# ppt0011/distributed_training

Measured on AMD Instinct MI355X. Metric: images/sec (node) ResNet-50 at 1/2/4/8 MI355X; grad-sync bus GB/s, higher is better.
Workload: dtype bf16

## Files before the change

distributed_training_amd/_lib.py:

```python
from __future__ import annotations

import ctypes
import os
import threading

import torch

LIB_PATH = os.environ.get(
    "GSYNC_LIB", os.path.join(os.path.dirname(os.path.abspath(__file__)), "lib", "libgsync.so")
)

GS_OK = 0
GS_EINVAL, GS_EHIP, GS_ERCCL, GS_ESTATE, GS_ENOMEM, GS_ENODEV = -1, -2, -3, -4, -5, -6
GS_F32, GS_BF16, GS_F16, GS_F64, GS_I64, GS_I32, GS_U8 = 0, 1, 2, 3, 4, 5, 6
GS_DEV_HOST, GS_DEV_HIP = 0, 1
GS_SUM, GS_PROD, GS_MAX, GS_MIN, GS_AVG = 0, 1, 2, 3, 4
GS_SCALE_NONE, GS_SCALE_MUL, GS_SCALE_DIV = 0, 1, 2
GS_PLAN_SLOTS = 5
GS_RED_GROUPS = 64
GS_RED_PARTIALS = 1024
GS_BKT_AUTO_COLLECTIVE = 1
GS_BKT_GRAD_VIEW = 2
GS_BKT_NO_SCALE = 4
GS_BKT_REDUCE_SCATTER = 8
GS_BKT_NO_UNPACK = 16
GS_LAYOUT_NCHW, GS_LAYOUT_NHWC = 0, 1
GS_OP_PACK, GS_OP_UNPACK, GS_OP_SCALE, GS_OP_SQNORM, GS_OP_UNSCALE, GS_OP_SGD, GS_OP_ADAM, GS_OP_SUM = 1, 2, 3, 4, 5, 6, 7, 8
GS_OP_LARS_NORM, GS_OP_LARS = 9, 10
GS_OP_LAMB_MOMENTS, GS_OP_LAMB = 11, 12
GS_OP_EMA = 13
GS_EMA_EMA, GS_EMA_SWA, GS_EMA_WARMUP = 0, 1, 2

_TORCH_TO_GS = {
    torch.float32: GS_F32,
    torch.bfloat16: GS_BF16,
    torch.float16: GS_F16,
    torch.float64: GS_F64,
    torch.int64: GS_I64,
    torch.int32: GS_I32,
    torch.uint8: GS_U8,
}

_c_int, _c_i64, _c_f, _c_d, _vp = ctypes.c_int, ctypes.c_int64, ctypes.c_float, ctypes.c_double, ctypes.c_void_p
_p_i64 = ctypes.POINTER(ctypes.c_int64)
_p_i32 = ctypes.POINTER(ctypes.c_int32)
_p_u8 = ctypes.POINTER(ctypes.c_uint8)
_p_vp = ctypes.POINTER(ctypes.c_void_p)
_p_f = ctypes.POINTER(ctypes.c_float)

SIGNATURES = {
    "gs_version": (_c_int, []),
    "gs_last_error": (ctypes.c_char_p, []),
    "gs_device_count": (_c_int, []),
    "gs_set_host_threads": (_c_int, [_c_int]),
    "gs_comm_unique_id_bytes": (_c_int, []),
    "gs_comm_get_unique_id": (_c_int, [_p_u8]),
    "gs_comm_create": (_c_int, [_c_int, _c_int, _p_u8, _c_int, _p_vp]),
    "gs_comm_create_ex": (_c_int, [_c_int, _c_int, _p_u8, _c_int, _c_int, _p_vp]),
    "gs_comm_destroy": (_c_int, [_vp]),
    "gs_comm_abort": (_c_int, [_vp]),
    "gs_comm_set_timeout": (_c_int, [_vp, _c_i64]),
    "gs_comm_status": (_c_int, [_vp, ctypes.c_char_p, _c_int]),
    "gs_comm_rank": (_c_int, [_vp]),
    "gs_comm_world": (_c_int, [_vp]),
    "gs_comm_stream": (_c_int, [_vp, _p_vp]),
    "gs_stream_wait": (_c_int, [_vp, _vp]),
    "gs_allreduce": (_c_int, [_vp, _vp, _vp, _c_i64, _c_int, _c_int, _vp]),
    "gs_reduce_scatter": (_c_int, [_vp, _vp, _vp, _c_i64, _c_int, _c_int, _vp]),
    "gs_all_gather": (_c_int, [_vp, _vp, _vp, _c_i64, _c_int, _vp]),
    "gs_broadcast": (_c_int, [_vp, _vp, _vp, _c_i64, _c_int, _c_int, _vp]),
    "gs_allreduce_marked": (_c_int, [_vp, _vp, _vp, _c_i64, _c_int, _c_int, _vp, _vp]),
    "gs_all_gather_marked": (_c_int, [_vp, _vp, _vp, _c_i64, _c_int, _vp, _vp]),
    "gs_plan_create": (_c_int, [_c_int, _c_int, _c_int, _p_i64, _c_i64, _p_vp]),
    "gs_plan_create_ex": (_c_int, [_c_int, _c_int, _c_int, _p_i64, _c_i64, _c_i64, _p_vp]),
    "gs_plan_destroy": (_c_int, [_vp]),
    "gs_plan_flat_numel": (_c_i64, [_vp]),
    "gs_plan_offsets": (_c_int, [_vp, _p_i64]),
    "gs_plan_n_tasks": (_c_int, [_vp]),
    "gs_plan_task_units": (_c_i64, [_vp]),
    "gs_plan_set_hyper_source": (_c_int, [_vp, _vp]),
    "gs_watchdog_pause": (_c_int, [_c_int]),
    "gs_adam_hyper": (_c_int, [_c_int, _vp, _vp, _c_d, _c_d, _c_d, _vp, _vp, _vp]),
    "gs_plan_timer_enable": (_c_int, [_vp, _c_int]),
    "gs_plan_timer_read": (_c_int, [_vp, _p_f, _p_i32, _c_int]),
    "gs_plan_set_ptrs": (_c_int, [_vp, _c_int, _p_vp, _vp]),
    "gs_pack": (_c_int, [_vp, _c_int, _c_int, _vp, _c_int, _c_f, _c_int, _vp]),
    "gs_unpack": (_c_int, [_vp, _vp, _c_int, _c_int, _c_int, _vp, _c_int, _vp]),
    "gs_unpack_check": (_c_int, [_vp, _vp, _c_int, _c_int, _c_int, _vp, _vp]),
    "gs_scale": (_c_int, [_vp, _c_int, _c_int, _c_f, _c_int, _vp]),
    "gs_sqnorm": (_c_int, [_vp, _c_int, _c_int, _vp, _c_int, _vp]),
    "gs_sum": (_c_int, [_vp, _c_int, _c_int, _vp, _c_int, _vp]),
    "gs_sqnorm_partial": (_c_int, [_vp, _c_int, _c_int, _vp]),
    "gs_plan_set_clip": (_c_int, [_vp, _vp, _c_f, _c_f, _c_f, _c_f, _vp]),
    "gs_plan_set_read_hint": (_c_int, [_vp, _c_int]),
    "gs_sqnorm_partial_out": (_c_int, [_vp, _c_int, _c_int, _vp, _p_i32, _vp]),
    "gs_plan_set_clip_groups": (_c_int, [_vp, _vp, ctypes.c_int32, _c_f, _c_f, _c_f, _c_f, _vp]),
    "gs_clip_scale": (_c_int, [_vp, _c_int, _c_int, _vp]),
    "gs_rng_state_bytes": (_c_int, []),
    "gs_rng_draw_u32": (_c_int, [_vp, _c_i64, _c_i64, _vp]),
    "gs_randperm": (_c_int, [ctypes.c_uint64, _c_i64, _vp]),
    "gs_distributed_sampler_indices": (_c_int, [_c_i64, _c_int, _c_int, _c_int, ctypes.c_uint64, _c_i64, _c_int,
                                                _vp, _c_i64, _p_i64]),
    "gs_crop_flip_params": (_c_int, [_vp, _c_i64, _c_int, _c_int, _c_int, _c_int, _c_int, _c_int, _vp, _c_i64,
                                     _vp]),
    "gs_image_augment": (_c_int, [_c_int, _c_int, _vp, _vp, _c_i64, _c_int, _c_int, _c_int, _c_int, _c_int, _c_int,
                                  _vp, _c_i64, _vp, _c_int, _c_int, _vp, _vp]),
    "gs_image_augment_mix": (_c_int, [_c_int, _c_int, _vp, _vp, _c_i64, _c_int, _c_int, _c_int, _c_int, _c_int, _c_int,
                                      _vp, _vp, _c_i64, _vp, _c_int, _c_int, _vp, _vp, _vp, _vp]),
    "gs_bn_bwd_partials": (_c_int, [_c_i64, _c_int]),
    "gs_bn_bwd_reduce": (_c_int, [_vp, _vp, _vp, _vp, _vp, _vp, _c_i64, _c_i64, _c_int, _vp]),
    "gs_bn_bwd_reduce_fork": (_c_int, [_vp, _vp, _vp, _vp, _vp, _vp, _vp, _c_i64, _c_i64, _c_int, _vp]),
    "gs_bn_bwd_dx": (_c_int, [_vp, _vp, _vp, _vp, _vp, _vp, _vp, _c_i64, _vp, _vp, _vp, _c_i64, _c_int, _vp]),
    "gs_add_relu_fwd": (_c_int, [_vp, _vp, _c_i64, _vp]),
    "gs_relu_maxpool_fwd": (_c_int, [_vp, _vp, _vp, _c_i64, _c_int, _c_int, _c_int, _vp]),
    "gs_maxpool_bwd": (_c_int, [_vp, _vp, _vp, _vp, _c_i64, _c_int, _c_int, _c_int, _vp]),
    "gs_relu_mask_fwd": (_c_int, [_vp, _vp, _c_i64, _vp]),
    "gs_add_relu_mask_fwd": (_c_int, [_vp, _vp, _vp, _c_i64, _vp]),
    "gs_relu_maxpool_mask_fwd": (_c_int, [_vp, _vp, _vp, _vp, _c_i64, _c_int, _c_int, _c_int, _vp]),
    "gs_bn_bwd_reduce_bits": (_c_int, [_vp, _vp, _vp, _vp, _vp, _vp, _c_i64, _c_i64, _c_int, _vp]),
    "gs_bn_bwd_reduce_fork_bits": (_c_int, [_vp, _vp, _vp, _vp, _vp, _vp, _vp, _c_i64, _c_i64, _c_int, _vp]),
    "gs_bn_bwd_dx_bits": (_c_int, [_vp, _vp, _vp, _vp, _vp, _vp, _vp, _c_i64, _vp, _vp, _vp, _c_i64, _c_int, _vp]),
    "gs_bn_infer_act": (_c_int, [_vp, _vp, _vp, _vp, _vp, _vp, _c_d, _c_int, _vp, _c_i64, _c_int, _vp]),
    "gs_bn_infer_relu_maxpool": (_c_int, [_vp, _vp, _vp, _vp, _vp, _c_d, _vp, _c_i64, _c_int, _c_int, _c_int, _vp]),
    "gs_eval_accumulate": (_c_int, [_c_int, _vp, _c_int, _vp, _c_i64, _c_i64, _c_i64, _c_i64, _p_i32, _c_int, _c_i64,
                                    _vp, _vp, _vp]),
    "gs_xent_fwd": (_c_int, [_c_int, _vp, _c_int, _vp, _c_i64, _c_i64, _c_i64, _c_i64, _c_f, _vp, _vp, _p_i32, _c_int,
                             _vp, _vp]),
    "gs_xent_bwd": (_c_int, [_c_int, _vp, _c_int, _vp, _c_i64, _c_i64, _c_i64, _c_i64, _c_f, _c_int, _vp, _vp, _vp, _vp,
                             _c_i64, _vp]),
    "gs_xent_mix_fwd": (_c_int, [_c_int, _vp, _c_int, _vp, _vp, _vp, _c_i64, _c_i64, _c_i64, _c_i64, _c_f, _vp, _vp,
                                 _p_i32, _c_int, _vp, _vp]),
    "gs_xent_mix_bwd": (_c_int, [_c_int, _vp, _c_int, _vp, _vp, _vp, _c_i64, _c_i64, _c_i64, _c_i64, _c_f, _c_int, _vp,
                                 _vp, _vp, _vp, _c_i64, _vp]),
    "gs_clip_coef":(_c_int, [_c_int, _vp, _c_f, _c_f, _vp, _vp, _vp]),
    "gs_unscale_check": (_c_int, [_vp, _c_int, _c_int, _vp, _vp, _vp]),
    "gs_sgd_step": (
        _c_int,
        [_vp, _c_int, _c_int, _c_d, _c_d, _c_d, _c_d, _c_int, _c_int, _c_int, _vp, _vp, _vp],
    ),
    "gs_adam_step": (
        _c_int,
        [_vp, _c_int, _c_int, _c_d, _c_d, _c_d, _c_d, _c_d, _c_int, _c_int, _c_d, _c_d, _vp, _vp, _vp],
    ),
    "gs_plan_set_adapt": (_c_int, [_vp, _p_i32]),
    "gs_lars_norms": (_c_int, [_vp, _c_int, _vp, _vp]),
    "gs_lars_step": (_c_int, [_vp, _c_int, _c_d, _c_d, _c_d, _c_d, _c_d, _vp, _vp, _vp, _vp]),
    "gs_lars_step_lowp": (_c_int, [_vp, _c_int, _c_int, _c_d, _c_d, _c_d, _c_d, _c_d, _vp, _vp, _vp, _vp]),
    "gs_lamb_step_lowp": (_c_int, [_vp, _c_int, _c_d, _c_d, _c_d, _c_d, _c_d, _c_d, _c_d, _vp, _vp, _vp]),
    "gs_lamb_moments": (_c_int, [_vp, _c_int, _c_d, _c_d, _c_d, _c_d, _c_d, _c_d, _vp, _vp, _vp, _vp]),
    "gs_lamb_step": (_c_int, [_vp, _c_d, _c_d, _c_d, _c_d, _c_d, _c_d, _c_d, _vp, _vp, _vp]),
    "gs_lamb_hyper": (_c_int, [_c_int, _vp, _vp, _c_d, _c_d, _c_int, _vp, _vp, _vp]),
    "gs_ema_step": (_c_int, [_vp, _c_int, _c_int, _c_d, _c_int, _vp]),
    "gs_ema_hyper": (_c_int, [_c_int, _vp, _c_int, _c_d, _vp, _vp]),
    "gs_compute_bucket_assignment": (
        _c_int,
        [_c_int, _p_i64, _p_i32, _p_i32, _c_int, _p_i64, _p_i32, _p_i32, _p_i32],
    ),
    "gs_bucketer_create": (
        _c_int,
        [_vp, _c_int, _c_int, _c_int, _p_i64, _c_int, _c_int, _p_i32, _p_i32, _c_int, _c_i64, _c_f, _c_int, _p_vp],
    ),
    "gs_bucketer_destroy": (_c_int, [_vp]),
    "gs_bucketer_bucket_numel": (_c_int, [_vp, _c_int, _p_i64]),
    "gs_bucketer_shard_numel": (_c_int, [_vp, _c_int, _p_i64]),
    "gs_bucketer_param_location": (_c_int, [_vp, _c_int, _p_i32, _p_i64]),
    "gs_bucketer_set_bucket_buffer": (_c_int, [_vp, _c_int, _vp]),
    "gs_bucketer_set_shard_buffer": (_c_int, [_vp, _c_int, _vp]),
    "gs_bucketer_prepare": (_c_int, [_vp, _vp]),
    "gs_bucketer_mark_ready": (_c_int, [_vp, _c_int, _vp, _vp, _p_i32, _p_i32]),
    "gs_bucketer_mark_unused": (_c_int, [_vp, _vp, _p_i32, _p_i32]),
    "gs_bucketer_finalize": (_c_int, [_vp, _vp]),
    "gs_bucketer_unpack_bucket": (_c_int, [_vp, _c_int, _vp]),
# ... 158 lines not shown
```

distributed_training_amd/csrc/gs_common.h:

```cpp
#pragma once

#include <cmath>
#include <cstdint>
#include <cstring>
#include <string>
#include <vector>

#include "../../include/gsync.h"
#include "gs_math.h"

namespace gs {

bool roctx_enabled();
void roctx_push(const char* name);
void roctx_pop();
struct GsRange {
  bool on;
  explicit GsRange(const char* name) : on(roctx_enabled()) {
    if (on) roctx_push(name);
  }
  ~GsRange() {
    if (on) roctx_pop();
  }
  GsRange(const GsRange&) = delete;
// ... 248 lines not shown
                        void* stream);
int host_eval_accumulate(const void* logits, int dt, const int64_t* labels, int64_t B, int K, int64_t row_stride,
                         int64_t n_valid, const EvalTopk& topk, int64_t ignore_index, void* ws, void* acc);

struct XentRow {
  float loss, m, logS;
  int32_t code;
};
static_assert(sizeof(XentRow) == 16, "XentRow layout");
struct XentRed {
  float loss_sum, loss_mean;
  int32_t counted, bad;
};
static_assert(sizeof(XentRed) == 16, "XentRed layout");
constexpr int kXentNone = 0, kXentMean = 1, kXentSum = 2;
GS_HD inline float xent_loss(float m, float logS, float zy, float T, int K, float eps) {
  const float nll = (m - zy) + logS;
  if (eps == 0.f) return nll;
  const float smooth = (m + logS) - T / static_cast<float>(K);
  return (1.f - eps) * nll + eps * smooth;
}
GS_HD inline XentRed xent_reduce(double total, int64_t counted, int64_t bad) {
  XentRed r;
  const float nanf32 = static_cast<float>(NAN);
  r.loss_sum = bad ? nanf32 : static_cast<float>(total);
  r.loss_mean = (bad || counted == 0) ? nanf32 : static_cast<float>(total / static_cast<double>(counted));
  r.counted = static_cast<int32_t>(counted);
  r.bad = static_cast<int32_t>(bad);
  return r;
}
GS_HD inline float xent_grad(float z, float m, float logS, float q, float c) {
  const float p = expf((z - m) - logS);
  return c * (p - q);
}
GS_HD inline int32_t xent_mix_code(int64_t a, int64_t b, float lam, int K, int64_t ignore_index) {
  if (a == ignore_index || b == ignore_index) return kEvalSkip;
  if (a < 0 || a >= K || b < 0 || b >= K || !(lam >= 0.f && lam <= 1.f)) return kEvalBad;
  return 0;
}
GS_HD inline bool xent_mix_one(int64_t a, int64_t b, float lam) { return lam == 1.f || a == b; }
GS_HD inline int64_t xent_mix_dominant(int64_t a, int64_t b, float lam) { return lam >= 0.5f ? a : b; }
GS_HD inline float xent_mix_loss(float m, float logS, float za, float zb, float lam, float T, int K, float eps) {
  const float lam1 = 1.f - lam;
  return lam * xent_loss(m, logS, za, T, K, eps) + lam1 * xent_loss(m, logS, zb, T, K, eps);
}
GS_HD inline float xent_mix_q(float eps, float w, float q_off) { return (1.f - eps) * w + q_off; }
int hip_xent_fwd(const void* logits, int dt, const int64_t* labels, int64_t B, int K, int64_t row_stride,
                 int64_t ignore_index, float eps, void* rows, void* red, const EvalTopk& topk, void* acc,
                 void* stream);
int hip_xent_bwd(const void* logits, int dt, const int64_t* labels, int64_t B, int K, int64_t row_stride, float eps,
                 int reduction, const void* rows, const void* red, const float* grad_out, void* dlogits,
                 int64_t d_row_stride, void* stream);
int hip_xent_mix_fwd(const void* logits, int dt, const int64_t* labels_a, const int64_t* labels_b, const float* lam,
                     int64_t B, int K, int64_t row_stride, int64_t ignore_index, float eps, void* rows, void* red,
                     const EvalTopk& topk, void* acc, void* stream);
int host_xent_mix_fwd(const void* logits, int dt, const int64_t* labels_a, const int64_t* labels_b, const float* lam,
                      int64_t B, int K, int64_t row_stride, int64_t ignore_index, float eps, void* rows, void* red,
                      const EvalTopk& topk, void* acc);
int hip_xent_mix_bwd(const void* logits, int dt, const int64_t* labels_a, const int64_t* labels_b, const float* lam,
                     int64_t B, int K, int64_t row_stride, float eps, int reduction, const void* rows, const void* red,
                     const float* grad_out, void* dlogits, int64_t d_row_stride, void* stream);
int host_xent_mix_bwd(const void* logits, int dt, const int64_t* labels_a, const int64_t* labels_b, const float* lam,
                      int64_t B, int K, int64_t row_stride, float eps, int reduction, const void* rows,
                      const void* red, const float* grad_out, void* dlogits, int64_t d_row_stride);

int comm_mark_take(gs_comm* c, void** ev);
bool stream_destroyed(void* stream);
int comm_mark_commit(gs_comm* c, void* ev, void* stream, const gs_plan* consumer);
void comm_forget_consumer(const gs_plan* consumer);

int hip_plan_upload_static(gs_plan* p);
int hip_plan_release(gs_plan* p);
int hip_plan_flush(gs_plan* p, void* stream);
bool stream_capturing(void* stream);
int hip_plan_timer_enable(gs_plan* p, int n_slots);
int hip_plan_timer_read(gs_plan* p, float* ms_out, int32_t* kind_out, int cap);
int hip_pack(gs_plan* p, int src_slot, int src_dt, void* flat, int flat_dt, float s, int mode,
             void* stream);
int hip_unpack(gs_plan* p, const void* flat, int flat_dt, int dst_slot, int dst_dt, float* sq,
               int acc, void* stream);
int hip_unpack_check(gs_plan* p, const void* flat, int flat_dt, int dst_slot, int dst_dt, float* found,
                     void* stream);
int hip_scale(gs_plan* p, int slot, int dt, float s, int mode, void* stream);
int hip_sqnorm(gs_plan* p, int slot, int dt, float* sq, int acc, void* stream);
int hip_sum(gs_plan* p, int slot, int dt, float* out, int acc, void* stream);
int hip_clip_coef(const float* sq, float max_norm, float eps, float* coef, float* norm,
                  void* stream);
int hip_unscale_check(gs_plan* p, int slot, int dt, const float* inv, float* found,
                      void* stream);
int hip_clip_scale(gs_plan* p, int slot, int dt, const ClipArgs& clip, void* stream);
int hip_sqnorm_partial(gs_plan* p, int slot, int dt, float* groups_out, int32_t* n_groups, void* stream);
const float* hip_plan_red_groups(const gs_plan* p);
float* hip_plan_red_scalar(const gs_plan* p);
int hip_sgd(gs_plan* p, int gdt, int ldt, const SgdHyper& h, const float* gs, const float* fi,
            const ClipArgs* clip, void* stream);
int hip_adam(gs_plan* p, int gdt, int ldt, const AdamHyper& h, const float* gs, const float* fi,
             const ClipArgs* clip, void* stream);
int hip_lars_set_adapt(gs_plan* p);
int hip_lars_norms(gs_plan* p, int gdt, float* norms, void* stream);
int hip_lars(gs_plan* p, int gdt, int ldt, const LarsHyper& h, const float* norms, const float* gs, const float* fi,
             void* stream);
int hip_lamb_moments(gs_plan* p, int gdt, const LambHyper& h, float* norms, const float* gs, const float* fi,
                     void* stream);
int hip_lamb(gs_plan* p, int ldt, const LambHyper& h, const float* norms, const float* fi, void* stream);
int hip_lamb_hyper(double* step, const double* lr, double beta1, double beta2, int bias_correction,
                   const float* found_inf, float* hyper, void* stream);
int hip_device_count();
int hip_memset_async(void* dst, int value, size_t bytes, void* stream);
int hip_stream_wait(void* waiter, void* signaler);

int host_pack(gs_plan* p, int src_slot, int src_dt, void* flat, int flat_dt, float s, int mode);
int host_unpack(gs_plan* p, const void* flat, int flat_dt, int dst_slot, int dst_dt, float* sq,
                int acc);
int host_unpack_check(gs_plan* p, const void* flat, int flat_dt, int dst_slot, int dst_dt, float* found);
int host_scale(gs_plan* p, int slot, int dt, float s, int mode);
int host_clip_scale(gs_plan* p, int slot, int dt, const ClipArgs& clip);
int host_sqnorm(gs_plan* p, int slot, int dt, float* sq, int acc);
int host_sum(gs_plan* p, int slot, int dt, float* out, int acc);
int host_clip_coef(const float* sq, float max_norm, float eps, float* coef, float* norm);
int host_unscale_check(gs_plan* p, int slot, int dt, const float* inv, float* found);
int host_sgd(gs_plan* p, int gdt, int ldt, const SgdHyper& h, const float* gs, const float* fi,
             const ClipArgs* clip);
int host_adam(gs_plan* p, int gdt, int ldt, const AdamHyper& h, const float* gs, const float* fi,
              const ClipArgs* clip);
int host_lars_norms(gs_plan* p, int gdt, float* norms);
int host_lars(gs_plan* p, int gdt, int ldt, const LarsHyper& h, const float* norms, const float* gs, const float* fi);
int host_lamb_moments(gs_plan* p, int gdt, const LambHyper& h, float* norms, const float* gs, const float* fi);
int host_lamb(gs_plan* p, int ldt, const LambHyper& h, const float* norms, const float* fi);
float host_clip_factor(const ClipArgs& c, const float* gs);
float host_wave_sum(const float* x, int n, int stride);
}
```

distributed_training_amd/csrc/gs_engine.h:

```cpp

#pragma once

#include <hip/hip_ext.h>
#include <hip/hip_runtime.h>

#include <algorithm>
#include <type_traits>
#include <cmath>
#include <cstdio>
#include <cstdlib>

#include "gs_common.h"

namespace gs {

namespace {

#define HIP_RET(expr)                                                                 \
  do {                                                                                \
    hipError_t _e = (expr);                                                           \
    if (_e != hipSuccess)                                                             \
      return fail(GS_EHIP, std::string(#expr " failed: ") + hipGetErrorString(_e));   \
  } while (0)

// ... 620 lines not shown
  static constexpr int kKind = GS_OP_SQNORM;
  struct Frag { float x[N]; };
  __device__ bool fast_ok(const TV& v) const { return v.vec(0); }
  template <bool F>
  __device__ void load(const TV& v, int64_t e0, uint32_t lo, Frag& f) const {
    ld<DT, N, F, NT>(v.ptr[0], e0, lo, v.numel, v.vec(0), f.x);
  }
  template <bool F>
  __device__ void apply(const TV&, int64_t, uint32_t, Frag& f, float& acc) const {
#pragma unroll
    for (int i = 0; i < N; ++i) acc = fmaf(f.x[i], f.x[i], acc);
  }
};

template <int N, int DT>
struct SumOp : SlotOpBase<N> {
  static constexpr int kG = GS_G_RED;
  static constexpr int kRed = 1;
  static constexpr int kRedGrid = 8192;
  static constexpr int kKind = GS_OP_SUM;
  struct Frag { float x[N]; };
  __device__ bool fast_ok(const TV& v) const { return v.vec(0); }
  template <bool F>
  __device__ void load(const TV& v, int64_t e0, uint32_t lo, Frag& f) const {
    ld<DT, N, F>(v.ptr[0], e0, lo, v.numel, v.vec(0), f.x);
  }
  template <bool F>
  __device__ void apply(const TV&, int64_t, uint32_t, Frag& f, float& acc) const {
#pragma unroll
    for (int i = 0; i < N; ++i) acc += f.x[i];
  }
};

template <int N, int DT>
struct UnscaleOp : SlotOpBase<N> {
  static constexpr int kG = GS_G_RED;
  static constexpr int kRed = 2;
  static constexpr int kRedGrid = 8192;
  static constexpr int kKind = GS_OP_UNSCALE;
  const float* inv;
  struct Frag { float x[N]; };
  __device__ bool fast_ok(const TV& v) const { return v.vec(0); }
  template <bool F>
  __device__ void load(const TV& v, int64_t e0, uint32_t lo, Frag& f) const {
    ld<DT, N, F>(v.ptr[0], e0, lo, v.numel, v.vec(0), f.x);
  }
  template <bool F>
  __device__ void apply(const TV& v, int64_t e0, uint32_t lo, Frag& f, float& acc) const {
#pragma unroll
    for (int i = 0; i < N; ++i)
      if ((F || e0 + lo + i < v.numel) && !isfinite(f.x[i])) acc = 1.f;
    if (inv) {
      const float s = *inv;
      if (s != 1.f) {
#pragma unroll
        for (int i = 0; i < N; ++i) f.x[i] = f.x[i] * s;
        st<DT, N, F>(v.ptr[0], e0, lo, v.numel, v.vec(0), f.x);
      }
    }
  }
};

template <int N, int DT, bool NT = false>
struct ClipScaleOp : SlotOpBase<N> {
  static constexpr int kG = GS_G_UNPACK;
  static constexpr int kKind = GS_OP_SCALE;
  ClipArgs clip{};
  float gsv = 1.f;
  struct Frag { float x[N]; };
  __device__ bool active() const { return gsv != 1.f; }
  __device__ bool fast_ok(const TV& v) const { return v.vec(0); }
  template <bool F>
  __device__ void load(const TV& v, int64_t e0, uint32_t lo, Frag& f) const {
    ld<DT, N, F, NT>(v.ptr[0], e0, lo, v.numel, v.vec(0), f.x);
  }
  template <bool F>
  __device__ void apply(const TV& v, int64_t e0, uint32_t lo, Frag& f, float&) const {
#pragma unroll
    for (int i = 0; i < N; ++i) f.x[i] = f.x[i] * gsv;
    st<DT, N, F>(v.ptr[0], e0, lo, v.numel, v.vec(0), f.x);
  }
};

template <int N, int GD, int LD, bool NTG = true>
struct SgdOp : OpBase<N> {
  static constexpr int kG = GS_G_SGD;
  static constexpr int kKind = GS_OP_SGD;
  SgdHyper h;
  const float* gscale;
  const float* found_inf;
  const float* hyper = nullptr;
  ClipArgs clip{};
  bool clip_on = false;
  bool use_gs = false;
  float gsv = 1.f;
  struct Frag { float p[N], g[N], b[N]; };
  __device__ bool active() const { return found_inf == nullptr || *found_inf == 0.f; }
  __device__ bool fast_ok(const TV& v) const {
    return v.vec(0) && v.vec(1) && (h.mom == 0.f || v.vec(2)) && (LD < 0 || v.vec(3));
  }
  template <bool F>
  __device__ void load(const TV& v, int64_t e0, uint32_t lo, Frag& f) const {
    ld<GS_F32, N, F>(v.ptr[0], e0, lo, v.numel, v.vec(0), f.p);
    ld<GD, N, F, NTG>(v.ptr[1], e0, lo, v.numel, v.vec(1), f.g);
    if (h.mom != 0.f && !h.first) ld<GS_F32, N, F>(v.ptr[2], e0, lo, v.numel, v.vec(2), f.b);
  }
  template <bool F>
  __device__ void apply(const TV& v, int64_t e0, uint32_t lo, Frag& f, float&) const {
#pragma unroll
    for (int i = 0; i < N; ++i) sgd_update(h, use_gs, gsv, f.g[i], &f.p[i], &f.b[i]);
    st<GS_F32, N, F>(v.ptr[0], e0, lo, v.numel, v.vec(0), f.p);
    if (h.mom != 0.f) st<GS_F32, N, F>(v.ptr[2], e0, lo, v.numel, v.vec(2), f.b);
    if constexpr (LD >= 0) st<LD, N, F>(v.ptr[3], e0, lo, v.numel, v.vec(3), f.p);
  }
};

template <int N, int GD, int LD = -1, bool NTG = false>
struct LarsOp : OpBase<N> {
  static constexpr int kG = GS_G_SGD;
  static constexpr int kKind = GS_OP_LARS;
  LarsHyper h;
  const float* norms;
  const int32_t* adapt;
  const float* gscale;
  const float* found_inf;
  const float* hyper = nullptr;
  bool use_gs = false;
  float gsv = 1.f;
  struct Frag { float p[N], g[N], b[N], slr, wd; };
  __device__ bool active() const { return found_inf == nullptr || *found_inf == 0.f; }
  __device__ bool fast_ok(const TV& v) const {
    return v.vec(0) && v.vec(1) && (h.mom == 0.f || v.vec(2)) && (LD < 0 || v.vec(3));
  }
  template <bool F>
  __device__ void load(const TV& v, int64_t e0, uint32_t lo, Frag& f) const {
    ld<GS_F32, N, F>(v.ptr[0], e0, lo, v.numel, v.vec(0), f.p);
    ld<GD, N, F, NTG>(v.ptr[1], e0, lo, v.numel, v.vec(1), f.g);
    if (h.mom != 0.f) ld<GS_F32, N, F>(v.ptr[2], e0, lo, v.numel, v.vec(2), f.b);
    const int t = v.pad;
    lars_coef(h, norms[2 * t], norms[2 * t + 1], adapt[t], use_gs, gsv, &f.slr, &f.wd);
  }
  template <bool F>
  __device__ void apply(const TV& v, int64_t e0, uint32_t lo, Frag& f, float&) const {
#pragma unroll
    for (int i = 0; i < N; ++i) lars_update(h, f.slr, f.wd, use_gs, gsv, f.g[i], &f.p[i], &f.b[i]);
    st<GS_F32, N, F>(v.ptr[0], e0, lo, v.numel, v.vec(0), f.p);
    if (h.mom != 0.f) st<GS_F32, N, F>(v.ptr[2], e0, lo, v.numel, v.vec(2), f.b);
    if constexpr (LD >= 0) st<LD, N, F>(v.ptr[3], e0, lo, v.numel, v.vec(3), f.p);
  }
};

#ifndef GS_G_LAMB
#define GS_G_LAMB 4
#endif
template <int N, int LD = -1>
struct LambOp : OpBase<N> {
  static constexpr int kG = GS_G_LAMB;
  static constexpr int kKind = GS_OP_LAMB;
  LambHyper h;
  const float* norms;
  const int32_t* adapt;
  const float* found_inf;
  const float* hyper = nullptr;
  struct Frag { float p[N], m[N], v[N], slr, wd; };
  __device__ bool active() const { return found_inf == nullptr || *found_inf == 0.f; }
  __device__ bool fast_ok(const TV& tv) const {
// ... 299 lines not shown
```

distributed_training_amd/csrc/gs_host.cpp:

```cpp
#include <algorithm>
#include <atomic>
#include <cmath>
#include <thread>

#include "gs_common.h"

namespace gs {
namespace {

template <int DT>
inline float ldT(const void* base, int64_t i) {
  if constexpr (DT == GS_F32) return static_cast<const float*>(base)[i];
  else return to_f32<DT>(static_cast<const uint16_t*>(base)[i]);
}
template <int DT>
inline void stT(void* base, int64_t i, float v) {
  if constexpr (DT == GS_F32) static_cast<float*>(base)[i] = v;
  else static_cast<uint16_t*>(base)[i] = from_f32<DT>(v);
}
inline void* slot(gs_plan* p, int s, int t) { return p->h_ptrs[static_cast<size_t>(s) * p->n + t]; }

int check_float(int dt) {
  if (!is_float_dtype(dt)) return fail(GS_EINVAL, "unsupported floating dtype");
  return GS_OK;
// ... 27 lines not shown

}

int host_pack(gs_plan* p, int src_slot, int src_dt, void* flat, int flat_dt, float s, int mode) {
  GS_DISPATCH_FLOAT(src_dt, SD, GS_DISPATCH_FLOAT(flat_dt, FD, {
    const int fsz = dtype_size(FD);
    for_ranges(p, [&](int t, int64_t i0, int64_t i1) {
      const void* src = slot(p, src_slot, t);
      void* dst = static_cast<char*>(flat) + p->off[t] * fsz;
      if (!src) {
        const float z = mode == GS_SCALE_MUL ? 0.f * s : (mode == GS_SCALE_DIV ? 0.f / s : 0.f);
        for (int64_t i = i0; i < i1; ++i) stT<FD>(dst, i, z);
      } else if (mode == GS_SCALE_MUL) {
        for (int64_t i = i0; i < i1; ++i) stT<FD>(dst, i, ldT<SD>(src, i) * s);
      } else if (mode == GS_SCALE_DIV) {
        for (int64_t i = i0; i < i1; ++i) stT<FD>(dst, i, round_to<FD>(ldT<SD>(src, i)) / s);
      } else {
        for (int64_t i = i0; i < i1; ++i) stT<FD>(dst, i, ldT<SD>(src, i));
      }
    });
  }));
  return GS_OK;
}

int host_unpack(gs_plan* p, const void* flat, int flat_dt, int dst_slot, int dst_dt, float* sq,
                int acc) {
  GS_DISPATCH_FLOAT(flat_dt, FD, GS_DISPATCH_FLOAT(dst_dt, DD, {
    const int fsz = dtype_size(FD);
    if (sq) {
      double total = 0.0;
      for (int t = 0; t < p->n; ++t) {
        const void* src = static_cast<const char*>(flat) + p->off[t] * fsz;
        void* dst = slot(p, dst_slot, t);
        if (dst == nullptr) continue;
        for (int64_t i = 0; i < p->numel[t]; ++i) {
          const float v = ldT<FD>(src, i);
          stT<DD>(dst, i, v);
          const float r = round_to<DD>(v);
          total += static_cast<double>(r) * r;
        }
      }
      sq[0] = acc ? sq[0] + static_cast<float>(total) : static_cast<float>(total);
    } else {
      for_ranges(p, [&](int t, int64_t i0, int64_t i1) {
        const void* src = static_cast<const char*>(flat) + p->off[t] * fsz;
        void* dst = slot(p, dst_slot, t);
        if (dst == nullptr) return;
        for (int64_t i = i0; i < i1; ++i) stT<DD>(dst, i, ldT<FD>(src, i));
      });
    }
  }));
  return GS_OK;
}

int host_unpack_check(gs_plan* p, const void* flat, int flat_dt, int dst_slot, int dst_dt, float* found) {
  std::atomic<int> bad{found[0] != 0.f ? 1 : 0};
  GS_DISPATCH_FLOAT(flat_dt, FD, GS_DISPATCH_FLOAT(dst_dt, DD, {
    const int fsz = dtype_size(FD);
    for_ranges(p, [&](int t, int64_t i0, int64_t i1) {
      const void* src = static_cast<const char*>(flat) + p->off[t] * fsz;
      void* dst = slot(p, dst_slot, t);
      if (dst == nullptr) return;
      int b = 0;
      for (int64_t i = i0; i < i1; ++i) {
        const float v = ldT<FD>(src, i);
        stT<DD>(dst, i, v);
        b |= !std::isfinite(round_to<DD>(v));
      }
      if (b) bad.store(1);
    });
  }));
  found[0] = bad.load() ? 1.f : 0.f;
  return GS_OK;
}

int host_scale(gs_plan* p, int s_, int dt, float s, int mode) {
  GS_DISPATCH_FLOAT(dt, DT, {
    for_ranges(p, [&](int t, int64_t i0, int64_t i1) {
      void* x = slot(p, s_, t);
      if (mode == GS_SCALE_DIV)
        for (int64_t i = i0; i < i1; ++i) stT<DT>(x, i, ldT<DT>(x, i) / s);
      else
        for (int64_t i = i0; i < i1; ++i) stT<DT>(x, i, ldT<DT>(x, i) * s);
    });
  });
  return GS_OK;
}

int host_clip_scale(gs_plan* p, int s_, int dt, const ClipArgs& clip) {
  const float cf = host_clip_factor(clip, nullptr);
  if (cf == 1.f) return GS_OK;
  return host_scale(p, s_, dt, cf, GS_SCALE_MUL);
}

int host_sqnorm(gs_plan* p, int s_, int dt, float* sq, int acc) {
  GS_DISPATCH_FLOAT(dt, DT, {
    double total = 0.0;
    for (int t = 0; t < p->n; ++t) {
      const void* x = slot(p, s_, t);
      for (int64_t i = 0; i < p->numel[t]; ++i) {
        const double v = ldT<DT>(x, i);
        total += v * v;
      }
    }
    sq[0] = acc ? sq[0] + static_cast<float>(total) : static_cast<float>(total);
  });
  return GS_OK;
}

int host_sum(gs_plan* p, int s_, int dt, float* out, int acc) {
  GS_DISPATCH_FLOAT(dt, DT, {
    double total = 0.0;
    for (int t = 0; t < p->n; ++t) {
      const void* x = slot(p, s_, t);
      for (int64_t i = 0; i < p->numel[t]; ++i) total += ldT<DT>(x, i);
    }
    out[0] = acc ? out[0] + static_cast<float>(total) : static_cast<float>(total);
  });
  return GS_OK;
}

int host_clip_coef(const float* sq, float max_norm, float eps, float* coef, float* norm) {
  const float nrm = sqrtf(sq[0]);
  if (norm) norm[0] = nrm;
  coef[0] = clip_coef(nrm, max_norm, eps, 0);
  return GS_OK;
}

int host_unscale_check(gs_plan* p, int s_, int dt, const float* inv, float* found) {
  std::atomic<int> bad{found[0] != 0.f ? 1 : 0};
  const bool scale = inv && inv[0] != 1.f;
  const float sc = scale ? inv[0] : 1.f;
  GS_DISPATCH_FLOAT(dt, DT, {
    for_ranges(p, [&](int t, int64_t i0, int64_t i1) {
      void* x = slot(p, s_, t);
      int b = 0;
      for (int64_t i = i0; i < i1; ++i) {
        const float v = ldT<DT>(x, i);
        b |= !std::isfinite(v);
        if (scale) stT<DT>(x, i, v * sc);
      }
      if (b) bad.store(1);
    });
  });
  found[0] = bad.load() ? 1.f : 0.f;
  return GS_OK;
}

float host_wave_sum(const float* x, int n, int stride) {
  float v[64], t[64];
  for (int l = 0; l < 64; ++l) {
    float a = 0.f;
    for (int j = l; j < n; j += 64) a = a + x[static_cast<int64_t>(j) * stride];
    v[l] = 0.f + a;
  }
  auto step = [&](auto src, unsigned row_mask) {
    for (int l = 0; l < 64; ++l) t[l] = ((row_mask >> (l >> 4)) & 1u) ? v[src(l)] : 0.f;
    for (int l = 0; l < 64; ++l) v[l] = v[l] + t[l];
  };
  static const int q1[4] = {1, 0, 3, 2}, q2[4] = {2, 3, 0, 1};
  step([](int l) { return (l & ~3) | q1[l & 3]; }, 0xFu);
  step([](int l) { return (l & ~3) | q2[l & 3]; }, 0xFu);
  step([](int l) { return (l & ~7) | (7 - (l & 7)); }, 0xFu);
  step([](int l) { return (l & ~15) | (15 - (l & 15)); }, 0xFu);
  step([](int l) { return (l & ~15) - 1; }, 0xAu);
  step([](int) { return 31; }, 0xCu);
// ... 431 lines not shown
```

distributed_training_amd/csrc/gs_kernels.hip:

```cpp

#include "gs_engine.h"

namespace gs {

int hip_device_count() {
  int n = 0;
  if (hipGetDeviceCount(&n) != hipSuccess) return 0;
  return n;
}

int hip_memset_async(void* dst, int value, size_t bytes, void* stream) {
  HIP_RET(hipMemsetAsync(dst, value, bytes, static_cast<hipStream_t>(stream)));
  return GS_OK;
}

int hip_stream_wait(void* waiter, void* signaler) {
  if (waiter == signaler) return GS_OK;
  hipEvent_t ev;
  HIP_RET(hipEventCreateWithFlags(&ev, hipEventDisableTiming));
  hipError_t e1 = hipEventRecord(ev, static_cast<hipStream_t>(signaler));
  hipError_t e2 = e1 == hipSuccess ? hipStreamWaitEvent(static_cast<hipStream_t>(waiter), ev, 0)
                                   : e1;
  (void)hipEventDestroy(ev);
  if (e2 != hipSuccess) return fail(GS_EHIP, std::string("stream wait: ") + hipGetErrorString(e2));
// ... 160 lines not shown
  HIP_RET(hipMemcpyAsync(p->d_table, stage, tb, hipMemcpyHostToDevice, s));
  HIP_RET(hipEventRecord(static_cast<hipEvent_t>(p->ring_events[k]), s));
  p->ring = (k + 1) & 3;
  p->dirty = false;
  return GS_OK;
}

constexpr int64_t kPackG2MaxChunks = 4096;

template <int SD, int FD, int MODE, bool NT>
static int pack_mode(gs_plan* p, int src_slot, void* flat, float s, void* stream) {
  if constexpr (FD == GS_F32) {
    if (static_cast<int64_t>(p->chunks.size()) <= kPackG2MaxChunks) {
      PackOp<kUnit, SD, FD, MODE, NT, true> op;
      op.slot = src_slot; op.flat = flat; op.flat_vec = flat_aligned(flat); op.s = s;
      return launch(p, op, stream);
    }
  }
  PackOp<kUnit, SD, FD, MODE, NT> op;
  op.slot = src_slot; op.flat = flat; op.flat_vec = flat_aligned(flat); op.s = s;
  return launch(p, op, stream);
}

template <bool NT>
static int pack_nt(gs_plan* p, int src_slot, int src_dt, void* flat, int flat_dt, float s, int mode,
                   void* stream) {
  GS_DISPATCH_FLOAT(src_dt, SD, GS_DISPATCH_FLOAT(flat_dt, FD, {
    switch (mode) {
      case GS_SCALE_NONE: return pack_mode<SD, FD, GS_SCALE_NONE, NT>(p, src_slot, flat, s, stream);
      case GS_SCALE_MUL: return pack_mode<SD, FD, GS_SCALE_MUL, NT>(p, src_slot, flat, s, stream);
      case GS_SCALE_DIV: return pack_mode<SD, FD, GS_SCALE_DIV, NT>(p, src_slot, flat, s, stream);
      default: return fail(GS_EINVAL, "gs_pack: unknown scale mode");
    }
  }));
  return GS_OK;
}

int hip_pack(gs_plan* p, int src_slot, int src_dt, void* flat, int flat_dt, float s, int mode,
             void* stream) {
  DeviceGuard g(p->device);
  return nt_read_once(p->elems * dtype_bytes(src_dt))
             ? pack_nt<true>(p, src_slot, src_dt, flat, flat_dt, s, mode, stream)
             : pack_nt<false>(p, src_slot, src_dt, flat, flat_dt, s, mode, stream);
}

template <int RED, bool NT>
static int unpack_nt(gs_plan* p, const void* flat, int flat_dt, int dst_slot, int dst_dt, float* red, int acc,
                     void* stream) {
  GS_DISPATCH_FLOAT(flat_dt, FD, GS_DISPATCH_FLOAT(dst_dt, DD, {
    UnpackOp<kUnit, FD, DD, RED, NT> op;
    op.want_red = red != nullptr; op.flat = flat; op.flat_vec = flat_aligned(flat); op.slot = dst_slot;
    return launch(p, op, stream, red, acc);
  }));
  return GS_OK;
}

int hip_unpack(gs_plan* p, const void* flat, int flat_dt, int dst_slot, int dst_dt, float* sq,
               int acc, void* stream) {
  DeviceGuard g(p->device);
  return nt_read_once(p->flat_numel * dtype_bytes(flat_dt))
             ? unpack_nt<1, true>(p, flat, flat_dt, dst_slot, dst_dt, sq, acc, stream)
             : unpack_nt<1, false>(p, flat, flat_dt, dst_slot, dst_dt, sq, acc, stream);
}

int hip_unpack_check(gs_plan* p, const void* flat, int flat_dt, int dst_slot, int dst_dt, float* found,
                     void* stream) {
  DeviceGuard g(p->device);
  return nt_read_once(p->flat_numel * dtype_bytes(flat_dt))
             ? unpack_nt<2, true>(p, flat, flat_dt, dst_slot, dst_dt, found, 1, stream)
             : unpack_nt<2, false>(p, flat, flat_dt, dst_slot, dst_dt, found, 1, stream);
}

int hip_scale(gs_plan* p, int slot, int dt, float s, int mode, void* stream) {
  DeviceGuard g(p->device);
  GS_DISPATCH_FLOAT(dt, DT, {
    ScaleOp<kUnit, DT> op;
    op.slot = slot; op.s = s; op.mode = mode;
    return launch(p, op, stream);
  });
  return GS_OK;
}

template <bool NT>
static int sqnorm_nt(gs_plan* p, int slot, int dt, float* sq, int acc, int groups_only, void* stream) {
  GS_DISPATCH_FLOAT(dt, DT, {
    SqnormOp<kUnit, DT, NT> op;
    op.slot = slot;
    return launch(p, op, stream, sq, acc, groups_only);
  });
  return GS_OK;
}
static int sqnorm_launch(gs_plan* p, int slot, int dt, float* sq, int acc, int groups_only, void* stream) {
  if (!nt_read_once(p->elems * dtype_bytes(dt), true, p->read_hint))
    return sqnorm_nt<false>(p, slot, dt, sq, acc, groups_only, stream);
  p->grads_read = false;
  return sqnorm_nt<true>(p, slot, dt, sq, acc, groups_only, stream);
}

int hip_sqnorm(gs_plan* p, int slot, int dt, float* sq, int acc, void* stream) {
  DeviceGuard g(p->device);
  return sqnorm_launch(p, slot, dt, sq, acc, 0, stream);
}

const float* hip_plan_red_groups(const gs_plan* p) {
  return p->d_partials + kGridLimit + kRedSyncWords + kRedSyncStride;
}
float* hip_plan_red_scalar(const gs_plan* p) { return p->d_partials + kGridLimit + kRedSyncWords; }

int hip_sqnorm_partial(gs_plan* p, int slot, int dt, float* groups_out, int32_t* n_groups, void* stream) {
  DeviceGuard g(p->device);
  const bool own = groups_out == nullptr;
  if (own) groups_out = const_cast<float*>(hip_plan_red_groups(p));
  if (!own && p->elems > 0 &&
      static_cast<int64_t>(p->chunks.size()) <= kRawChunksMax) {
    GS_TRY_RET(sqnorm_launch(p, slot, dt, groups_out, 0, 2, stream));
    if (n_groups) *n_groups = p->red_groups;
    p->red_valid = false;
    p->red_groups = 0;
    return GS_OK;
  }
  const int cap = std::min(p->grid_cap, red_grid_cap(SqnormOp<kUnit, GS_F32>::kRedGrid));
  const bool groups = p->elems > 0 &&
                      red_fuse_groups() > 0 && cap <= kRedFuseMaxGrid;
  if (groups) {
    GS_TRY_RET(sqnorm_launch(p, slot, dt, groups_out, 0, 1, stream));
    if (n_groups) *n_groups = p->red_groups;
    return GS_OK;
  }
  p->red_groups = 0;
  if (n_groups) *n_groups = 1;
  GS_TRY_RET(sqnorm_launch(p, slot, dt, hip_plan_red_scalar(p), 0, 0, stream));
  if (!own) {
    HIP_RET(hipMemsetAsync(groups_out, 0, GS_RED_PARTIALS * sizeof(float), static_cast<hipStream_t>(stream)));
    HIP_RET(hipMemcpyAsync(groups_out, hip_plan_red_scalar(p), sizeof(float), hipMemcpyDeviceToDevice,
                           static_cast<hipStream_t>(stream)));
  }
  return GS_OK;
}

int hip_sum(gs_plan* p, int slot, int dt, float* out, int acc, void* stream) {
  DeviceGuard g(p->device);
  GS_DISPATCH_FLOAT(dt, DT, {
    SumOp<kUnit, DT> op;
    op.slot = slot;
    return launch(p, op, stream, out, acc);
  });
  return GS_OK;
}

int hip_clip_coef(const float* sq, float max_norm, float eps, float* coef, float* norm,
                  void* stream) {
  hipLaunchKernelGGL(clip_coef_kernel, dim3(1), dim3(64), 0, static_cast<hipStream_t>(stream),
                     sq, max_norm, eps, coef, norm);
  HIP_RET(hipGetLastError());
  return GS_OK;
}

__global__ void adam_hyper_kernel(double* step, const double* lr, double beta1, double beta2, double wd,
                                  const float* found_inf, float* hyper) {
  if (threadIdx.x == 0) adam_hyper_update(step, lr, beta1, beta2, wd, found_inf, hyper);
}

int hip_adam_hyper(double* step, const double* lr, double beta1, double beta2, double wd,
                   const float* found_inf, float* hyper, void* stream) {
  hipLaunchKernelGGL(adam_hyper_kernel, dim3(1), dim3(64), 0, static_cast<hipStream_t>(stream), step, lr,
                     beta1, beta2, wd, found_inf, hyper);
// ... 47 lines not shown
```

distributed_training_amd/csrc/gs_plan.cpp:

```cpp
#include <algorithm>
#include <cstdlib>
#include <map>
#include <new>

#include <rocprofiler-sdk-roctx/roctx.h>

#include "gs_common.h"

namespace gs {

static thread_local std::string g_last_error;

bool roctx_enabled() {
  static const bool on = [] {
    const char* e = std::getenv("GSYNC_ROCTX");
    return e && std::atoi(e) != 0;
  }();
  return on;
}
void roctx_push(const char* name) { roctxRangePushA(name); }
void roctx_pop() { roctxRangePop(); }

void set_error(const std::string& msg) { g_last_error = msg; }
int fail(int code, const std::string& msg) {
// ... 180 lines not shown
  std::copy(p->off.begin(), p->off.end(), out);
  return GS_OK;
}

int gs_plan_n_tasks(gs_plan* p) { return p ? p->n_tasks : -1; }

int64_t gs_plan_task_units(gs_plan* p) { return p ? p->task_units : -1; }

int gs_plan_timer_enable(gs_plan* p, int n_slots) {
  GS_CHECK_ARG(p != nullptr, "gs_plan_timer_enable: NULL plan");
  GS_CHECK_ARG(n_slots >= 0 && n_slots <= 4096, "gs_plan_timer_enable: n_slots out of [0, 4096]");
  if (p->kind != GS_DEV_HIP) return fail(GS_EINVAL, "gs_plan_timer_enable: host plans have no launch timer");
  return hip_plan_timer_enable(p, n_slots);
}

int gs_plan_timer_read(gs_plan* p, float* ms_out, int32_t* kind_out, int cap) {
  GS_CHECK_ARG(p != nullptr && (cap == 0 || ms_out != nullptr), "gs_plan_timer_read: NULL argument");
  if (p->kind != GS_DEV_HIP) return fail(GS_EINVAL, "gs_plan_timer_read: host plans have no launch timer");
  return hip_plan_timer_read(p, ms_out, kind_out, cap);
}

int gs_plan_set_ptrs(gs_plan* p, int slot, void* const* ptrs, void* ) {
  GS_CHECK_ARG(p != nullptr, "gs_plan_set_ptrs: NULL plan");
  GS_CHECK_ARG(slot >= 0 && slot < GS_PLAN_SLOTS, "gs_plan_set_ptrs: slot out of range");
  GS_CHECK_ARG(p->n == 0 || ptrs != nullptr, "gs_plan_set_ptrs: NULL ptrs");
  void** row = p->h_ptrs.data() + static_cast<size_t>(slot) * p->n;
  for (int t = 0; t < p->n; ++t) {
    if (row[t] != ptrs[t]) {
      row[t] = ptrs[t];
      const uint32_t bit = 1u << slot;
      const bool al = (reinterpret_cast<uintptr_t>(ptrs[t]) & 15u) == 0;
      p->h_align[t] = al ? (p->h_align[t] | bit) : (p->h_align[t] & ~bit);
      p->dirty = true;
    }
  }
  return GS_OK;
}

#define PLAN_OK(p) GS_CHECK_ARG((p) != nullptr, "NULL plan")
#define SLOT_OK(s) GS_CHECK_ARG((s) >= 0 && (s) < GS_PLAN_SLOTS, "slot out of range")

int gs_pack(gs_plan* p, int src_slot, int src_dtype, void* flat, int flat_dtype, float scale,
            int scale_mode, void* stream) {
  GsRange range("gs_pack");
  PLAN_OK(p);
  SLOT_OK(src_slot);
  GS_CHECK_ARG(flat != nullptr || p->flat_numel == 0, "gs_pack: NULL flat buffer");
  GS_CHECK_ARG(scale_mode >= GS_SCALE_NONE && scale_mode <= GS_SCALE_DIV, "gs_pack: bad scale_mode");
  if (p->kind == GS_DEV_HOST) return host_pack(p, src_slot, src_dtype, flat, flat_dtype, scale, scale_mode);
  return hip_pack(p, src_slot, src_dtype, flat, flat_dtype, scale, scale_mode, stream);
}

int gs_unpack(gs_plan* p, const void* flat, int flat_dtype, int dst_slot, int dst_dtype,
              float* sqnorm_dev, int accumulate, void* stream) {
  GsRange range("gs_unpack");
  PLAN_OK(p);
  SLOT_OK(dst_slot);
  GS_CHECK_ARG(flat != nullptr || p->flat_numel == 0, "gs_unpack: NULL flat buffer");
  if (p->kind == GS_DEV_HOST)
    return host_unpack(p, flat, flat_dtype, dst_slot, dst_dtype, sqnorm_dev, accumulate);
  return hip_unpack(p, flat, flat_dtype, dst_slot, dst_dtype, sqnorm_dev, accumulate, stream);
}

int gs_unpack_check(gs_plan* p, const void* flat, int flat_dtype, int dst_slot, int dst_dtype,
                    float* found_inf, void* stream) {
  GsRange range("gs_unpack_check");
  PLAN_OK(p);
  SLOT_OK(dst_slot);
  GS_CHECK_ARG(flat != nullptr || p->flat_numel == 0, "gs_unpack_check: NULL flat buffer");
  GS_CHECK_ARG(found_inf != nullptr, "gs_unpack_check: NULL found_inf");
  if (p->kind == GS_DEV_HOST) return host_unpack_check(p, flat, flat_dtype, dst_slot, dst_dtype, found_inf);
  return hip_unpack_check(p, flat, flat_dtype, dst_slot, dst_dtype, found_inf, stream);
}

int gs_scale(gs_plan* p, int slot, int dtype, float s, int scale_mode, void* stream) {
  GsRange range("gs_scale");
  PLAN_OK(p);
  SLOT_OK(slot);
  GS_CHECK_ARG(scale_mode == GS_SCALE_MUL || scale_mode == GS_SCALE_DIV, "gs_scale: bad scale_mode");
  if (p->kind == GS_DEV_HOST) return host_scale(p, slot, dtype, s, scale_mode);
  return hip_scale(p, slot, dtype, s, scale_mode, stream);
}

int gs_sqnorm(gs_plan* p, int slot, int dtype, float* sqnorm_dev, int accumulate, void* stream) {
  GsRange range("gs_sqnorm");
  PLAN_OK(p);
  SLOT_OK(slot);
  GS_CHECK_ARG(sqnorm_dev != nullptr, "gs_sqnorm: NULL output");
  p->grads_read = slot == 1;
  if (p->kind == GS_DEV_HOST) return host_sqnorm(p, slot, dtype, sqnorm_dev, accumulate);
  return hip_sqnorm(p, slot, dtype, sqnorm_dev, accumulate, stream);
}

int gs_sqnorm_partial(gs_plan* p, int slot, int dtype, void* stream) {
  GsRange range("gs_sqnorm_partial");
  PLAN_OK(p);
  SLOT_OK(slot);
  p->red_valid = true;
  p->grads_read = slot == 1;
  if (p->kind == GS_DEV_HOST) {
    p->red_groups = 0;
    return host_sqnorm(p, slot, dtype, &p->h_red, 0);
  }
  return hip_sqnorm_partial(p, slot, dtype, nullptr, nullptr, stream);
}

int gs_sqnorm_partial_out(gs_plan* p, int slot, int dtype, float* groups_out, int32_t* n_groups,
                          void* stream) {
  GsRange range("gs_sqnorm_partial_out");
  PLAN_OK(p);
  SLOT_OK(slot);
  GS_CHECK_ARG(groups_out != nullptr && n_groups != nullptr, "gs_sqnorm_partial_out: NULL argument");
  p->red_valid = true;
  p->grads_read = slot == 1;
  if (p->kind == GS_DEV_HOST) {
    p->red_groups = 0;
    GS_TRY_RET(host_sqnorm(p, slot, dtype, &p->h_red, 0));
    groups_out[0] = p->h_red;
    std::fill(groups_out + 1, groups_out + GS_RED_PARTIALS, 0.f);
    *n_groups = 1;
    return GS_OK;
  }
  return hip_sqnorm_partial(p, slot, dtype, groups_out, n_groups, stream);
}

int gs_plan_set_read_hint(gs_plan* p, int hint) {
  PLAN_OK(p);
  GS_CHECK_ARG(hint >= 0 && hint <= 2, "gs_plan_set_read_hint: hint 0, 1 or 2");
  p->read_hint = hint;
  return GS_OK;
}

int gs_plan_set_clip(gs_plan* p, const float* sqnorm_dev, float max_norm, float eps, float sq_mul,
                     float coef_mul, float* out_dev) {
  PLAN_OK(p);
  if (!(max_norm > 0.f)) {
    p->clip_on = false;
    return GS_OK;
  }
  GS_CHECK_ARG(eps >= 0.f, "gs_plan_set_clip: eps < 0");
  p->clip_on = true;
  p->clip_own = sqnorm_dev == nullptr;
  p->clip = ClipArgs{sqnorm_dev, 0, 1, max_norm, eps, sq_mul, coef_mul, out_dev};
  return GS_OK;
}

int gs_plan_set_clip_groups(gs_plan* p, const float* groups_dev, int32_t n_groups, float max_norm,
                            float eps, float sq_mul, float coef_mul, float* out_dev) {
  PLAN_OK(p);
  if (!(max_norm > 0.f)) {
    p->clip_on = false;
    return GS_OK;
  }
  GS_CHECK_ARG(groups_dev != nullptr, "gs_plan_set_clip_groups: NULL group sums");
  GS_CHECK_ARG(n_groups >= 1 && n_groups <= GS_RED_PARTIALS, "gs_plan_set_clip_groups: n_groups out of 1..GS_RED_PARTIALS");
  GS_CHECK_ARG(eps >= 0.f, "gs_plan_set_clip_groups: eps < 0");
  p->clip_on = true;
  p->clip_own = false;
  p->clip = ClipArgs{groups_dev, n_groups, 1, max_norm, eps, sq_mul, coef_mul, out_dev};
  return GS_OK;
}

static int plan_clip(gs_plan* p, ClipArgs* c, const ClipArgs** out) {
  *out = nullptr;
  if (!p->clip_on) return GS_OK;
  *c = p->clip;
// ... 370 lines not shown
```

distributed_training_amd/csrc/gs_torch_hook.cpp:

```cpp
#include <pybind11/pybind11.h>
#include <pybind11/stl.h>
#include <torch/csrc/autograd/engine.h>
#include <torch/csrc/autograd/function.h>
#include <torch/csrc/autograd/function_hook.h>
#include <torch/csrc/autograd/variable.h>
#include <torch/csrc/utils/pybind.h>

#include <ATen/hip/impl/HIPStreamMasqueradingAsCUDA.h>
#include <c10/hip/HIPStream.h>

#include <algorithm>
#include <memory>
#include <stdexcept>
#include <string>
#include <vector>

#include "../../include/gsync.h"

namespace py = pybind11;
using torch::autograd::Node;
using torch::autograd::variable_list;

namespace {

// ... 119 lines not shown
    }
    const int bk = bucket_of_[i];
    held_[bk].push_back(g);
    p.mutable_grad() = at::Tensor();
    int32_t n_ready = 0;
    const int rc = gs_bucketer_mark_ready(b_, i, g.data_ptr(), stream_, ready_.data(), &n_ready);
    if (rc < 0) throw std::runtime_error(std::string("gs_bucketer_mark_ready: ") + gs_last_error());
    for (int k = 0; k < n_ready; ++k) {
      auto& hs = held_[ready_[k]];
      if (comm_stream_ != nullptr) {
        const c10::Stream cs = c10::hip::getStreamFromExternalMasqueradingAsCUDA(
            static_cast<hipStream_t>(comm_stream_), static_cast<c10::DeviceIndex>(device_));
        for (auto& t : hs) t.record_stream(cs);
      }
      hs.clear();
    }
  }

  void set_mark_unused(bool on) { mark_unused_ = on; }

  void finalize() {
    if (mark_unused_) {
      int32_t n_ready = 0;
      const int ru = gs_bucketer_mark_unused(b_, stream_, ready_.data(), &n_ready);
      if (ru < 0) {
        in_backward_ = false;
        finalize_queued_ = false;
        pinned_.clear();
        throw std::runtime_error(std::string("gs_bucketer_mark_unused: ") + gs_last_error());
      }
    }
    const int rc = gs_bucketer_finalize(b_, stream_);
    in_backward_ = false;
    finalize_queued_ = false;
    pinned_.clear();
    if (rc < 0) throw std::runtime_error(std::string("gs_bucketer_finalize: ") + gs_last_error());
    std::string err;
    const PyGILState_STATE st = PyGILState_Ensure();
    PyObject* r = PyObject_CallObject(on_finalize_, nullptr);
    if (r == nullptr) {
      PyObject *t, *v, *tb;
      PyErr_Fetch(&t, &v, &tb);
      PyObject* sv = v ? PyObject_Str(v) : nullptr;
      const char* msg = sv ? PyUnicode_AsUTF8(sv) : nullptr;
      err = msg ? msg : "error in the DDP finalize callback";
      Py_XDECREF(sv);
      Py_XDECREF(t);
      Py_XDECREF(v);
      Py_XDECREF(tb);
      PyErr_Clear();
    }
    Py_XDECREF(r);
    PyGILState_Release(st);
    if (!err.empty()) throw std::runtime_error(err);
  }

  std::vector<int> order() const { return order_; }
  bool in_backward() const { return in_backward_; }
  bool finalize_queued() const { return finalize_queued_; }
  uintptr_t stream() const { return reinterpret_cast<uintptr_t>(stream_); }

 private:
  std::vector<at::Tensor> params_;
  int device_;
  PyObject* on_finalize_;
  std::vector<std::weak_ptr<Node>> accs_;
  std::vector<std::shared_ptr<Node>> pinned_;
  std::vector<uintptr_t> keys_;
  bool active_ = false;
  std::vector<std::vector<int64_t>> dense_strides_;
  std::vector<char> dense_seen_;
  gs_bucketer* b_ = nullptr;
  std::vector<int32_t> ready_;
  void* stream_ = nullptr;
  bool in_backward_ = false, finalize_queued_ = false, record_order_ = false;
  bool release_ = false;
  bool mark_unused_ = false;
  std::vector<int> bucket_of_;
  std::vector<std::vector<at::Tensor>> held_;
  void* comm_stream_ = nullptr;
  std::vector<int> order_;
};

variable_list MarkReady::operator()(const variable_list& outputs, const variable_list& ) {
  owner->on_grad(index);
  return outputs;
}

}

PYBIND11_MODULE(_gshook, m) {
  m.doc() = "libgsync DDP gradient hooks in C++ (AccumulateGrad post-hooks -> gs_bucketer_mark_ready)";
  py::class_<Hooks, std::shared_ptr<Hooks>>(m, "Hooks")
      .def(py::init<std::vector<at::Tensor>, int, py::function, bool>(), py::arg("params"), py::arg("device"),
           py::arg("on_finalize"), py::arg("release") = false)
      .def("attach", &Hooks::attach)
      .def("detach", &Hooks::detach)
      .def("attached", &Hooks::attached)
      .def("set_bucketer", &Hooks::set_bucketer, py::arg("handle"), py::arg("n_buckets"),
           py::arg("bucket_of") = std::vector<int>(), py::arg("comm_stream") = 0)
      .def("set_mark_unused", &Hooks::set_mark_unused)
      .def("prepare", &Hooks::prepare)
      .def("order", &Hooks::order)
      .def("in_backward", &Hooks::in_backward)
      .def("finalize_queued", &Hooks::finalize_queued)
      .def("stream", &Hooks::stream);
}
```

distributed_training_amd/ddp.py:

```python
from __future__ import annotations

import ctypes
import os
import sys
from contextlib import contextmanager
from dataclasses import dataclass
from enum import Enum, auto
from typing import Any, Callable

import torch
import torch.distributed as dist
import torch.nn as nn
from torch.distributed.algorithms.join import Join, Joinable, JoinHook

from . import _lib as L
from .comm import get_communicator
from .multi_tensor import TensorListPlan, dense_like_param, is_dense

DEFAULT_FIRST_BUCKET_BYTES = getattr(dist, "_DEFAULT_FIRST_BUCKET_BYTES", 1024 * 1024)
BUCKET_ALIGN_ELEMS = 64


def compute_bucket_assignment_by_size(tensors, size_limits, order=None):
    n = len(tensors)
    nbytes = L.i64_array([t.numel() * t.element_size() for t in tensors])
    keys = []
    key_ids: dict = {}
    for t in tensors:
        k = (t.dtype, t.device)
        keys.append(key_ids.setdefault(k, len(key_ids)))
    limits = [int(min(x, 2**62)) for x in size_limits]
    bucket_of = (ctypes.c_int32 * max(1, n))()
    members = (ctypes.c_int32 * max(1, n))()
    counts = (ctypes.c_int32 * max(1, n))()
    nb = L.check(
        L.lib().gs_compute_bucket_assignment(
            n, nbytes, L.i32_array(keys), None if order is None else L.i32_array(order), len(limits),
            L.i64_array(limits), bucket_of, members, counts),
        "gs_compute_bucket_assignment",
    )
    out, pos = [], 0
    for b in range(nb):
        out.append([int(members[pos + k]) for k in range(counts[b])])
        pos += counts[b]
    return out


def split_last_bucket(buckets, nbytes, cap):
    if not buckets:
        return buckets
    last = list(buckets[-1])
    tail, size = [], 0
    while last and (not tail or size + nbytes[last[-1]] <= cap):
        i = last.pop()
        tail.insert(0, i)
        size += nbytes[i]
    out = [list(b) for b in buckets[:-1]]
    if last:
        out.append(last)
    out.append(tail)
    return out


def xgmi_bucket_caps(allreduce_time, world: int, sizes_mib=(1, 4, 16, 64), efficiency: float = 0.85) -> dict:
    f = 2.0 * (world - 1) / world
    pts = [(m * 1024 * 1024, allreduce_time(m * 1024 * 1024)) for m in sizes_mib]
    n = len(pts)
    sx = sum(p[0] for p in pts)
    sy = sum(p[1] for p in pts)
    sxx = sum(p[0] * p[0] for p in pts)
    sxy = sum(p[0] * p[1] for p in pts)
    beta = (n * sxy - sx * sy) / max(1e-30, n * sxx - sx * sx)
    alpha = max(0.0, (sy - beta * sx) / n)
    if beta <= 0:
        beta = pts[-1][1] / pts[-1][0]
    bus = f / beta
    cap = efficiency / (1 - efficiency) * alpha * bus / f
    cap = int(min(256 * 2**20, max(4 * 2**20, cap)))
    last = int(min(cap, max(256 * 1024, alpha * bus / f)))
    return {"points": [{"bytes": b, "ms": t * 1e3, "bus_GBps": b * f / t / 1e9} for b, t in pts],
            "alpha_us": alpha * 1e6, "bus_GBps": bus / 1e9, "bucket_cap_bytes": cap, "last_bucket_cap_bytes": last,
            "efficiency": efficiency}


def _as_words(t: torch.Tensor):
    if not t.is_contiguous():
        return None
    if t.dtype in (torch.float32, torch.bfloat16, torch.float16):
        return t
    if t.element_size() in (4, 8) and t.dtype != torch.complex64:
        return t.reshape(-1).view(torch.float32)
    return None


class GradBucket:

    def __init__(self, index, buffer, params, offsets, is_last):
        self._index = index
# ... 192 lines not shown
        self.device_ids = device_ids if device_ids is None else [torch.device(d).index if not isinstance(d, int) else d for d in device_ids]
        self.output_device = output_device
        dtypes = {p.dtype for p in self._params}
        if not all(dt.is_floating_point for dt in dtypes):
            raise NotImplementedError(f"gradient sync needs floating parameters, got {dtypes}")
        self._bucket_dtype_override = bucket_dtype
        self._grad_dtype = self._params[0].dtype if len(dtypes) == 1 else None
        self._bucket_dtype = bucket_dtype if bucket_dtype is not None else self._grad_dtype
        if self.device.type == "cuda":
            self._dev_index = self.device.index if self.device.index is not None else torch.cuda.current_device()
            if not L.available():
                raise L.GsyncUnavailable(L._load_error)
        else:
            self._dev_index = 0
        self._backend = dist.get_backend(self.process_group)

        self._comm = None
        self._own_comm = False
        if self.device.type == "cuda" and collective != "process_group" and self._backend == "nccl":
            pg = None if self.process_group is dist.group.WORLD else self.process_group
            if rccl_max_ctas:
                from .comm import Communicator

                self._comm = Communicator(pg, torch.device("cuda", self._dev_index), max_ctas=int(rccl_max_ctas))
                self._own_comm = True
            else:
                self._comm = get_communicator(pg, torch.device("cuda", self._dev_index))
        self._comm_hook: tuple[Any, Callable] | None = None
        self._buffers_plan = None
        self._sqnorm_target: torch.Tensor | None = None
        self._sqnorm_valid = False
        self._sqnorm_versions = None
        self._found_inf_target: torch.Tensor | None = None
        self._found_inf_valid = False

        self._debug_sums = None
        if os.environ.get("GSYNC_DEBUG", "0") not in ("", "0"):
            self._debug_sums = torch.zeros(0)

        if init_sync:
            self._verify_param_shape_across_processes()
            self._sync_module_states()

        if bucket_policy not in ("torch", "xgmi"):
            raise ValueError(f"bucket_policy must be 'torch' or 'xgmi', got {bucket_policy!r}")
        self.bucket_policy = bucket_policy
        self._last_bucket_cap = None if last_bucket_cap_mb is None else int(last_bucket_cap_mb * 1024 * 1024)
        self._xgmi_calibration = None
        if bucket_policy == "xgmi" and self.world_size > 1:
            cal = xgmi_bucket_caps(self._calib_allreduce, self.world_size)
            self._xgmi_calibration = cal
            if bucket_cap_mb is None:
                self.bucket_bytes_cap = cal["bucket_cap_bytes"]
            if last_bucket_cap_mb is None:
                self._last_bucket_cap = cal["last_bucket_cap_bytes"]

        if static_graph or not find_unused_parameters:
            limits = [sys.maxsize]
        elif self.bucket_bytes_cap_default:
            limits = [DEFAULT_FIRST_BUCKET_BYTES, self.bucket_bytes_cap]
        else:
            limits = [self.bucket_bytes_cap]
        buckets = compute_bucket_assignment_by_size(self._params, limits)
        self._bucketer = self._make_bucketer(list(reversed(buckets)))
        self._has_rebuilt_buckets = False
        self._ready_order: list[int] = []
        self._in_backward = False
        self._finalize_queued = False
        self._stream = None
        self._pending: dict[int, Any] = {}
        self._num_iterations = 0
        self._capture_local: dict | None = None
        self._used_local = [0] * len(self._params) if find_unused_parameters else None
        self._ready_now: list = []
        self._overlap: dict | None = None
        self._param_index = {id(p): i for i, p in enumerate(self._params)}
        self._hook_handles = []
        self._native = _make_native_hooks(self) if self.device.type == "cuda" else None
        self._native_on = False
        if self._native is not None:
            self._native.set_bucketer(self._bucketer.handle.value, len(self._bucketer.buckets))
            self._native.set_mark_unused(bool(self.static_graph))
        self._set_native(self._native_ok())

    def _flags(self):
        flags = 0
        if self._comm is not None and self._comm_hook is None:
            flags |= L.GS_BKT_AUTO_COLLECTIVE
        if self.gradient_as_bucket_view:
            flags |= L.GS_BKT_GRAD_VIEW
        if self._comm_hook is not None:
            flags |= L.GS_BKT_NO_SCALE
        return flags

    def _make_bucketer(self, buckets):
        old = getattr(self, "_bucketer", None)
        if old is not None:
            old.close()
        b = _Bucketer(self, buckets, self._flags())
        self._div_factor = float(self.world_size)
        t = getattr(self, "_found_inf_target", None)
        if t is not None:
            L.check(L.lib().gs_bucketer_set_found_inf(b.handle, t.data_ptr()), "gs_bucketer_set_found_inf")
        if getattr(self, "_debug_sums", None) is not None:
            self._debug_sums = torch.zeros(3 * len(buckets), dtype=torch.float32, device=self.device)
            L.check(L.lib().gs_bucketer_set_debug(b.handle, self._debug_sums.data_ptr()), "gs_bucketer_set_debug")
        lvl = getattr(self, "_timeline", None)
        if lvl is not None:
            L.check(L.lib().gs_bucketer_set_timeline(b.handle, lvl), "gs_bucketer_set_timeline")
        if getattr(self, "_overlap", None) is not None:
            self._overlap["per_bucket"] = {}
        if getattr(self, "_native", None) is not None:
            self._native.set_bucketer(b.handle.value, len(buckets))
        return b

    def _native_ok(self) -> bool:
        return (self._native is not None and bool(self._bucketer.flags & L.GS_BKT_AUTO_COLLECTIVE)
                and not self.find_unused_parameters and self._overlap is None and self._comm_hook is None
                and self._capture_local is None)

    def _set_native(self, on: bool):
        if on:
            for h in self._hook_handles:
                h.remove()
            self._hook_handles = []
            self._native.attach()
        else:
            if self._native is not None:
                self._native.detach()
            if not self._hook_handles:
                self._hook_handles = [p.register_post_accumulate_grad_hook(self._make_hook(i))
                                      for i, p in enumerate(self._params)]
        self._native_on = on

    def _native_finalized(self):
        if self._record_order:
            self._ready_order = list(self._native.order())
        if self._post_bwd_futs:
            self._wait_post_backward_futures()
        self._found_inf_valid = self._found_inf_target is not None
        self._sqnorm_valid = self._sqnorm_fusable()
        self._sqnorm_versions = self._grad_versions() if self._sqnorm_valid else None
        if self.gradient_as_bucket_view:
            b = self._bucketer
            for i, p in enumerate(self._params):
                if p.grad is not None:
                    view = b.bucket_view(i)
                    if p.grad.data_ptr() != view.data_ptr():
                        p.grad = view
        self._in_backward = False
        self._finalize_queued = False
        self._num_iterations += 1

    def _calib_allreduce(self, nbytes: int, iters: int = 4) -> float:
        import time

        n = max(1, nbytes // 4)
        on_dev = self._comm is not None or self._backend == "nccl"
        buf = torch.zeros(n, dtype=torch.float32, device=self.device if on_dev else "cpu")
        ts = []
        for it in range(iters + 1):
            if on_dev:
                torch.cuda.synchronize(self.device)
            self._ctl_barrier()
            t0 = time.perf_counter()
            if self._comm is not None:
                self._comm.all_reduce(buf, stream=L.stream_ptr(self.device))
                torch.cuda.synchronize(self.device)
            else:
                dist.all_reduce(buf, group=self.process_group)
                if on_dev:
                    torch.cuda.synchronize(self.device)
            if it:
                ts.append(time.perf_counter() - t0)
        ts.sort()
        return float(self._ctl_all_reduce(torch.tensor([ts[len(ts) // 2]], dtype=torch.float64), "max").item())

    _CTL_OPS = {"sum": dist.ReduceOp.SUM, "min": dist.ReduceOp.MIN, "max": dist.ReduceOp.MAX}

    def _ctl_device(self):
        return self.device if (self._comm is not None or self._backend == "nccl") else torch.device("cpu")

    def _ctl_all_reduce(self, t: torch.Tensor, op: str = "sum") -> torch.Tensor:
        t = t.to(self._ctl_device())
        if self._comm is not None:
            self._comm.all_reduce(t, op=op, stream=L.stream_ptr(self.device))
        else:
            dist.all_reduce(t, op=self._CTL_OPS[op], group=self.process_group)
        return t

    def _ctl_broadcast(self, t: torch.Tensor) -> torch.Tensor:
        t = t.to(self._ctl_device())
        if self._comm is not None:
            self._comm.broadcast(t, root=0, stream=L.stream_ptr(self.device))
        else:
            dist.broadcast(t, src=dist.get_global_rank(self.process_group, 0)
                           if self.process_group is not dist.group.WORLD else 0, group=self.process_group)
# ... 89 lines not shown

    @torch.no_grad()
    def _sync_module_states(self):
        seen, params = set(), []
        for n, p in self.module.named_parameters():
            if n in self.parameters_to_ignore:
                continue
            if id(p) not in seen:
                seen.add(id(p))
                params.append(p.detach())
        self._broadcast_tensors(params + self._module_buffers())

    @torch.no_grad()
    def _sync_buffers(self, root: int = 0):
        if self.buffer_hook is not None:
            self._run_buffer_hook()
            return
        bufs = self._module_buffers()
        if self.world_size == 1 or not bufs:
            return
        key = tuple(id(t) for t in bufs)
        if self._buffers_plan is None or self._buffers_plan[0] != key:
            groups: dict = {}
            others = []
            for t in bufs:
                w = _as_words(t)
                if w is None:
                    others.append(t)
                else:
                    groups.setdefault(w.dtype, []).append(w)
            plans = []
            for dt, ws in groups.items():
                plan = TensorListPlan([w.numel() for w in ws], self.device, align=BUCKET_ALIGN_ELEMS)
                flat = torch.zeros(plan.flat_numel, dtype=dt, device=self.device)
                plan.set_ptrs(0, ws)
                plans.append((plan, ws, dt, flat))
            self._buffers_plan = (key, plans, others)
        _, plans, others = self._buffers_plan
        for plan, ws, dt, flat in plans:
            plan.set_ptrs(0, ws)
            if self.rank == root:
                plan.pack(0, dt, flat)
            self._bcast_flat(flat, root)
            if self.rank != root:
                plan.unpack(flat, 0, dt)
        if others:
            flat = torch.cat([t.reshape(-1) for t in others])
            self._bcast_flat(flat, root)
            if self.rank != root:
                off = 0
                for t in others:
                    t.copy_(flat[off:off + t.numel()].view_as(t))
                    off += t.numel()

    def _will_sync_module_buffers(self):
        return ((self.world_size > 1 or self.buffer_hook is not None) and self.require_forward_param_sync
                and self.broadcast_buffers and len(self._module_buffers()) != 0)

    def forward(self, *inputs, **kwargs):
        L.flush_deferred()
        if self._comm is not None:
            self._comm.check()
        grad_sync = torch.is_grad_enabled() and self.require_backward_grad_sync
        work = Join.notify_join_context(self)
        if grad_sync:
            self._maybe_rebuild_buckets()
        if work is not None and not self._divide_by_initial_world_size:
            work.wait()
            self._set_div_factor(float(work.result()[0].item()))
        elif self._div_factor != self.world_size and not self._join_config.enable:
            self._set_div_factor(float(self.world_size))
        joining = self._join_config.enable
        bh = self.buffer_hook
        sync_bufs = self._will_sync_module_buffers()
        post_fwd = bh is not None and bh.buffer_comm_hook_location == _BufferCommHookLocation.POST_FORWARD
        if sync_bufs and not post_fwd:
            self._sync_buffers(self._find_common_rank(self.rank, True) if joining else 0)
        if joining:
            self._check_global_requires_backward_grad_sync(is_joined_rank=False)
        if self.device_ids:
            dev = torch.device(self.device_type, self.device_ids[0])
            inputs = tuple(x.to(dev, non_blocking=True) if isinstance(x, torch.Tensor) else x for x in inputs)
            kwargs = {k: (v.to(dev, non_blocking=True) if isinstance(v, torch.Tensor) else v) for k, v in kwargs.items()}
        output = self.module(*inputs, **kwargs)
        if sync_bufs and post_fwd:
            self._sync_buffers()
        if grad_sync:
            self.require_forward_param_sync = True
            self._prepare_for_backward()
        else:
            self.require_forward_param_sync = False
            self._found_inf_valid = False
            self._sqnorm_valid = False
        return output

    def _prepare_for_backward(self):
        want = self._native_ok()
        if want != self._native_on:
            self._set_native(want)
        if self._native_on and self._in_backward and self._native.finalize_queued():
            self._finalize_queued = True
        if self._in_backward and self._finalize_queued:
            raise RuntimeError(
                "Expected to have finished reduction in the prior iteration before starting a new one. "
                "This error indicates that your module has parameters that were not used in producing loss.")
        sq = self._sqnorm_target
        if self._found_inf_target is not None:
            self._found_inf_target.zero_()
        self._found_inf_valid = False
        self._sqnorm_valid = False
        L.check(L.lib().gs_bucketer_prepare(self._bucketer.handle, None if sq is None else sq.data_ptr()),
                "gs_bucketer_prepare")
        self._in_backward = True
        self._finalize_queued = False
        self._pending = {}
        self._record_order = not self._has_rebuilt_buckets and (self.static_graph or not self.find_unused_parameters)
        self._ready_now = []
        if self._record_order:
            self._ready_order = []
        if self._native_on:
            self._native.prepare(self._record_order)

    @contextmanager
    def no_sync(self):
        old = self.require_backward_grad_sync
        self.require_backward_grad_sync = False
        try:
            yield
        finally:
            self.require_backward_grad_sync = old

    def _make_hook(self, idx):
        dense_strides = [None]

        def hook(param):
            if not self._in_backward:
                if self._used_local is not None:
                    self._used_local[idx] = 1
                return
            if not self._finalize_queued:
                self._finalize_queued = True
                self._stream = L.stream_ptr(self.device)
                torch.autograd.Variable._execution_engine.queue_callback(self._finalize_backward)
            if self._record_order:
                self._ready_order.append(idx)
            if self._used_local is not None:
                self._used_local[idx] = 1
                self._ready_now.append(idx)
            g = param.grad
            ps = param.stride()
            if g.stride() != ps or dense_strides[0] != ps:
                if not dense_like_param(g, param):
                    dense = torch.empty_like(param)
                    dense.copy_(g)
                    param.grad = g = dense
                elif is_dense(param):
                    dense_strides[0] = ps
            cap = self._capture_local
            if cap is not None and idx in cap:
                cap[idx] = g.detach().clone()
            b = self._bucketer
            rc = b._mark(b.handle, idx, g.data_ptr(), self._stream, b._ready, b._n_ready_ref)
            if rc < 0:
                L.check(rc, "gs_bucketer_mark_ready")
            if b._n_ready.value:
                ready = [b._ready[k] for k in range(b._n_ready.value)]
                if not (b.flags & L.GS_BKT_AUTO_COLLECTIVE):
                    self._launch_external(ready)
                elif self._overlap is not None:
                    self._overlap_step(ready)

        return hook

    def _launch_external(self, bucket_ids):
        b = self._bucketer
        nb = len(b.buckets)
        for bi in bucket_ids:
            buf = b.buffers[bi]
            if self._comm_hook is not None:
                state, hook = self._comm_hook
                gb = GradBucket(bi, buf, [self._params[i] for i in b.buckets[bi]], b.offsets_in_bucket[bi],
                                bi == nb - 1)
                self._pending[bi] = ("fut", hook(state, gb))
            elif self._comm is not None:
                self._comm.all_reduce(buf, stream=L.stream_ptr(self.device))
                self._pending[bi] = ("done", None)
            elif buf.is_cuda and self._backend == "gloo":
                host = buf.to("cpu")
                self._pending[bi] = ("host", (host, dist.all_reduce(host, group=self.process_group,
                                                                    async_op=True)))
            else:
                self._pending[bi] = ("work", dist.all_reduce(buf, group=self.process_group, async_op=True))

    def _finalize_backward(self):
        b = self._bucketer
        if self.find_unused_parameters:
            fired = set(self._ready_now)
            for i, p in enumerate(self._params):
                if i not in fired and p.grad is not None:
                    g = p.grad
                    if not dense_like_param(g, p):
                        dense = torch.empty_like(p)
                        dense.copy_(g)
                        p.grad = g = dense
                    L.check(L.lib().gs_bucketer_mark_ready(b.handle, i, g.data_ptr(), self._stream, b._ready,
                                                           ctypes.byref(b._n_ready)), "gs_bucketer_mark_ready")
                    self._dispatch_ready(b)
            L.check(L.lib().gs_bucketer_mark_unused(b.handle, self._stream, b._ready, ctypes.byref(b._n_ready)),
                    "gs_bucketer_mark_unused")
            self._dispatch_ready(b)
        elif self.static_graph:
            L.check(L.lib().gs_bucketer_mark_unused(b.handle, self._stream, b._ready, ctypes.byref(b._n_ready)),
                    "gs_bucketer_mark_unused")
            self._dispatch_ready(b)
        for bi in sorted(self._pending):
            kind, obj = self._pending[bi]
            if kind == "work":
                obj.wait()
            elif kind == "host":
                host, work = obj
                work.wait()
# ... 8 lines not shown
        if self._post_bwd_futs:
            self._wait_post_backward_futures()
        L.check(L.lib().gs_bucketer_finalize(b.handle, self._stream), "gs_bucketer_finalize")
        if self._overlap is not None and not (b.flags & L.GS_BKT_AUTO_COLLECTIVE):
            self._overlap_step(range(len(b.buckets)))
        self._found_inf_valid = self._found_inf_target is not None
        self._sqnorm_valid = self._sqnorm_fusable()
        self._sqnorm_versions = self._grad_versions() if self._sqnorm_valid else None
        if self.find_unused_parameters:
            if self.world_size > 1:
                self._grads_of_locally_unused()
            self._used_local = [0] * len(self._params)
        if self.gradient_as_bucket_view:
            for i, p in enumerate(self._params):
                if p.grad is not None:
                    view = b.bucket_view(i)
                    if p.grad.data_ptr() != view.data_ptr():
                        p.grad = view
        self._in_backward = False
        self._finalize_queued = False
        self._num_iterations += 1

    def _dispatch_ready(self, b):
        if b._n_ready.value:
            ready = [b._ready[k] for k in range(b._n_ready.value)]
            if not (b.flags & L.GS_BKT_AUTO_COLLECTIVE):
                self._launch_external(ready)
            elif self._overlap is not None:
                self._overlap_step(ready)

    def _grads_of_locally_unused(self):
        glob = self._ctl_all_reduce(torch.tensor(self._used_local, dtype=torch.int32), "max").tolist()
        b = self._bucketer
        made = []
        for i, p in enumerate(self._params):
            if glob[i] and not self._used_local[i]:
                view = b.bucket_view(i)
                if view.dtype != p.dtype:
                    p.grad = view.to(p.dtype, memory_format=torch.preserve_format)
                elif self.gradient_as_bucket_view:
                    p.grad = view
                else:
                    p.grad = view.clone(memory_format=torch.preserve_format)
                made.append(p.grad)
        if made:
            self._check_extra_grads(made)

    def _check_extra_grads(self, grads):
        if self._found_inf_target is None and self._sqnorm_target is None:
            return
        by_dtype: dict = {}
        for g in grads:
            by_dtype.setdefault(g.dtype, []).append(g)
        cache = self.__dict__.setdefault("_extra_plans", {})
        for dt, gs in by_dtype.items():
            key = (dt,) + tuple(g.numel() for g in gs)
            plan = cache.get(key)
            if plan is None:
                plan = cache[key] = TensorListPlan([g.numel() for g in gs], self.device)
            plan.set_ptrs(0, gs)
            if self._found_inf_target is not None:
                plan.unscale_check(0, dt, None, self._found_inf_target)
            if self._sqnorm_target is not None:
                plan.sqnorm(0, dt, self._sqnorm_target, accumulate=True)

    def _maybe_rebuild_buckets(self):
        if self._has_rebuilt_buckets or not (self.static_graph or not self.find_unused_parameters):
            return
        if len(self._ready_order) != len(self._params) or self._num_iterations == 0:
            return
        limits = [self.first_bucket_bytes_cap, self.bucket_bytes_cap]
        buckets = compute_bucket_assignment_by_size(self._params, limits, order=self._ready_order)
        if self._last_bucket_cap is not None:
            buckets = split_last_bucket(buckets, [p.numel() * p.element_size() for p in self._params],
                                        self._last_bucket_cap)
        buckets = self._sync_bucket_indices(buckets)
        if self.gradient_as_bucket_view:
            for p in self._params:
                if p.grad is not None:
                    p.grad = p.grad.clone()
        self._bucketer = self._make_bucketer(buckets)
        self._has_rebuilt_buckets = True
        self._ready_order = []

    def _sync_bucket_indices(self, buckets):
        if self.world_size == 1:
            return buckets
        n = len(self._params)
        flat = [len(buckets)] + [len(b) for b in buckets] + [i for b in buckets for i in b]
        flat += [0] * (2 * n + 1 - len(flat))
        v = self._ctl_broadcast(torch.tensor(flat, dtype=torch.int64)).tolist()
        nb = v[0]
        counts = v[1:1 + nb]
        out, pos = [], 1 + nb
        for c in counts:
            out.append(v[pos:pos + c])
            pos += c
        return out

    def _overlap_step(self, bucket_ids):
        ov = self._overlap
        main = ov["opt"]
        hyper = {k: v for k, v in main.param_groups[0].items() if k != "params"}
        for bi in bucket_ids:
            bo = ov["per_bucket"].get(bi)
            if bo is None:
                members = [self._params[i] for i in self._bucketer.buckets[bi] if id(self._params[i]) in ov["ids"]]
                bo = ov["cls"](members, *ov["args"], **ov["kwargs"]) if members else False
                ov["per_bucket"][bi] = bo
            if not bo:
                continue
            bo.state = main.state
            bo.param_groups[0].update(hyper)
            ptr = ctypes.c_void_p()
            L.check(L.lib().gs_bucketer_bucket_stream(self._bucketer.handle, bi, ctypes.byref(ptr)),
                    "gs_bucketer_bucket_stream")
            if ptr.value:
                st = ov["streams"].get(ptr.value)
                if st is None:
                    st = ov["streams"][ptr.value] = torch.cuda.ExternalStream(ptr.value, device=self.device)
                with torch.cuda.stream(st):
                    self._step_bucket(bi, bo)
            else:
                self._step_bucket(bi, bo)

    def _step_bucket(self, bi, bo):
        tmp = []
        for p in bo.param_groups[0]["params"]:
            if p.grad is None:
                i = self._param_index[id(p)]
                view = self._bucketer.bucket_view(i)
                p.grad = view if view.dtype == p.dtype else view.to(p.dtype, memory_format=torch.preserve_format)
                tmp.append(p)
        bo.step()
        for p in tmp:
            p.grad = None

    def _register_fused_optim(self, optim: type, *args, optim_params=None, **kwargs):
        import inspect

        from .optim import FusedAdam, FusedAdamW, FusedSGD

        if self._overlap is not None:
            raise RuntimeError("_register_fused_optim should only be called once on a DDP instance")
        if self._comm_hook is not None:
            raise RuntimeError("_register_fused_optim and register_comm_hook do not compose (as in torch)")
        table = {torch.optim.SGD: FusedSGD, torch.optim.Adam: FusedAdam, torch.optim.AdamW: FusedAdamW,
                 FusedSGD: FusedSGD, FusedAdam: FusedAdam, FusedAdamW: FusedAdamW}
        cls = next((table[c] for c in inspect.getmro(optim) if c in table), None)
        if cls is None:
            raise RuntimeError(f"{optim} does not support overlapped DDP (SGD, Adam, AdamW)")
        if kwargs.get("max_grad_norm"):
            raise RuntimeError("overlapped optimizer: a global-norm clip needs every bucket before any update")
        if self._found_inf_target is not None:
            raise RuntimeError("overlapped optimizer: AMP loss scaling needs the overflow check of every bucket "
                               "before any update (torch's overlapped optimizer has no GradScaler path either)")
        params = list(optim_params) if optim_params is not None else list(self._params)
        opt = cls(params, *args, **kwargs)
        self._overlap = {"cls": cls, "args": args, "kwargs": kwargs, "opt": opt, "ids": {id(p) for p in params},
                         "per_bucket": {}, "streams": {}}
        self._overlapped_optimizer = opt

    def register_comm_hook(self, state: object, hook: Callable):
        if self._comm_hook is not None:
            raise RuntimeError("register_comm_hook or register_builtin_comm_hook can only be called once.")
        if self._overlap is not None:
# ... 118 lines not shown
        if self._overlap is not None:
            raise NotImplementedError("join() with the overlapped optimizer")
        return Join([self], enable, throw_on_early_termination,
                    divide_by_initial_world_size=divide_by_initial_world_size)

    def join_hook(self, **kwargs) -> JoinHook:
        self._divide_by_initial_world_size = kwargs.get("divide_by_initial_world_size", True)
        return _DDPJoinHook(self)

    def _set_div_factor(self, div: float):
        if div != self._div_factor:
            L.check(L.lib().gs_bucketer_set_div_factor(self._bucketer.handle, float(div)),
                    "gs_bucketer_set_div_factor")
            self._div_factor = div

    @property
    def join_device(self) -> torch.device:
        return self.device

    @property
    def join_process_group(self):
        return self.process_group

    def _find_common_rank(self, input_rank: int, rank_cond: bool) -> int:
        r = self._ctl_all_reduce(torch.tensor([input_rank if rank_cond else -1], dtype=torch.int64), "max")
        v = int(r.item())
        if v < 0:
            raise ValueError("join: no rank qualified as the common rank")
        return v

    def _check_global_requires_backward_grad_sync(self, is_joined_rank: bool):
        t = torch.tensor([1.0 if (not is_joined_rank and self.require_backward_grad_sync) else 0.0])
        t = self._ctl_all_reduce(t, "sum")
        return bool(t.item() != 0) if is_joined_rank else None

    def _match_all_reduce_for_bwd_pass(self):
        b = self._bucketer
        nb = len(b.buckets)
        for bi, buf in enumerate(b.buffers):
            z = torch.zeros_like(buf)
            if self._comm_hook is not None:
                state, hook = self._comm_hook
                hook(state, GradBucket(bi, z, [self._params[i] for i in b.buckets[bi]], b.offsets_in_bucket[bi],
                                       bi == nb - 1)).wait()
            elif self._comm is not None:
                self._comm.all_reduce(z, stream=L.stream_ptr(self.device))
            elif z.is_cuda and self._backend == "gloo":
                dist.all_reduce(z.cpu(), group=self.process_group)
            else:
                dist.all_reduce(z, group=self.process_group)

    def _sync_final_model(self, is_last_joiner: bool):
        root = self._find_common_rank(self.rank, is_last_joiner)
        seen, ts = set(), []
        for n, p in self.module.named_parameters():
            if n not in self.parameters_to_ignore and id(p) not in seen:
                seen.add(id(p))
                ts.append(p.detach())
        if self.broadcast_buffers:
            ts += self._module_buffers()
        with torch.no_grad():
            self._broadcast_tensors(ts, root)

    @staticmethod
    def _set_params_and_buffers_to_ignore_for_model(module, params_and_buffers_to_ignore):
        module._ddp_params_and_buffers_to_ignore = params_and_buffers_to_ignore
        for name, param in module.named_parameters():
            if name in params_and_buffers_to_ignore:
                param._ddp_ignored = True
        for name, buffer in module.named_buffers():
            if name in params_and_buffers_to_ignore:
                buffer._ddp_ignored = True

    def bucket_indices(self):
        return [list(b) for b in self._bucketer.buckets]

    def close(self):
        for h in getattr(self, "_hook_handles", []):
            try:
                h.remove()
            except Exception:
                pass
        self._hook_handles = []
        if getattr(self, "_native", None) is not None:
            self._native.detach()
            self._native_on = False
        b = getattr(self, "_bucketer", None)
        if b is not None:
            if self.gradient_as_bucket_view:
                for p in self._params:
                    if p.grad is not None:
                        p.grad = p.grad.clone()
            b.close()
        if getattr(self, "_own_comm", False) and self._comm is not None:
            self._comm.close()
            self._own_comm = False

    def __del__(self):
        for h in getattr(self, "_hook_handles", []):
            try:
                h.remove()
            except Exception:
                pass
        nat = getattr(self, "_native", None)
        if nat is not None:
            nat.detach()


class _DDPJoinHook(JoinHook):

    def __init__(self, ddp):
        self.ddp = ddp
        super().__init__()

    def main_hook(self):
        d = self.ddp
        d._maybe_rebuild_buckets()
        bh = d.buffer_hook
        post_fwd = bh is not None and bh.buffer_comm_hook_location == _BufferCommHookLocation.POST_FORWARD
        sync_bufs = d._will_sync_module_buffers()
        if sync_bufs and not post_fwd:
            d._sync_buffers(d._find_common_rank(d.rank, False))
        should_sync = d._check_global_requires_backward_grad_sync(is_joined_rank=True)
        if sync_bufs and post_fwd:
            d._sync_buffers()
            d._wait_post_backward_futures()
        d.require_forward_param_sync = should_sync
        if not should_sync:
            return
        d._match_all_reduce_for_bwd_pass()
        if d.find_unused_parameters:
            d._ctl_all_reduce(torch.zeros(len(d._params), dtype=torch.int32), "max")

    def post_hook(self, is_last_joiner: bool):
        self.ddp._sync_final_model(is_last_joiner)


DDP = DistributedDataParallel
```

distributed_training_amd/multi_tensor.py:

```python
from __future__ import annotations

import ctypes
from typing import Sequence

import torch

from . import _lib as L

UPDATE_TASK_UNITS = 512


def update_task_units(device) -> int:
    return UPDATE_TASK_UNITS if torch.device(device).type == "cuda" else 0


class TensorListPlan:
    def __init__(self, numels: Sequence[int], device: torch.device, align: int = 0, task_units: int = 0):
        self.device = torch.device(device)
        self.kind = L.GS_DEV_HIP if self.device.type == "cuda" else L.GS_DEV_HOST
        self.numels = [int(n) for n in numels]
        self.n = len(self.numels)
        dev_index = self.device.index if self.device.index is not None else (
            torch.cuda.current_device() if self.kind == L.GS_DEV_HIP else 0
        )
# ... 30 lines not shown
        if self.kind == L.GS_DEV_HOST:
            L.lib().gs_set_host_threads(torch.get_num_threads())
        return L.stream_ptr(self.device)

    def set_ptrs(self, slot: int, tensors_or_ptrs):
        ptrs = tuple(
            (t if isinstance(t, int) or t is None else t.data_ptr()) for t in tensors_or_ptrs
        )
        if len(ptrs) != self.n:
            raise ValueError(f"plan has {self.n} tensors, got {len(ptrs)} pointers")
        if self._slot_cache.get(slot) == ptrs:
            return
        for t, n in zip(tensors_or_ptrs, self.numels):
            if isinstance(t, torch.Tensor) and t.numel() != n:
                raise ValueError(f"plan tensor of {n} elements bound to a tensor of {t.numel()}")
        L.check(L.lib().gs_plan_set_ptrs(self.handle, slot, L.ptr_array(ptrs), None), "gs_plan_set_ptrs")
        self._slot_cache[slot] = ptrs

    @property
    def n_tasks(self) -> int:
        return int(L.lib().gs_plan_n_tasks(self.handle))

    @property
    def task_units(self) -> int:
        return int(L.lib().gs_plan_task_units(self.handle))

    def set_hyper_source(self, hyper: torch.Tensor | None):
        if hyper is not None:
            if hyper.dtype != torch.float32 or not hyper.is_contiguous() or hyper.numel() < 3:
                raise ValueError("hyper source: contiguous fp32 tensor of >= 3 elements")
            if (hyper.device.type == "cuda") != (self.kind == L.GS_DEV_HIP):
                raise ValueError("hyper source must live where the plan runs")
        L.check(L.lib().gs_plan_set_hyper_source(self.handle, None if hyper is None else hyper.data_ptr()),
                "gs_plan_set_hyper_source")
        self._hyper = hyper

    def timer_enable(self, n_slots: int = 256):
        L.check(L.lib().gs_plan_timer_enable(self.handle, int(n_slots)), "gs_plan_timer_enable")

    def timer_read(self, cap: int = 4096, kind: int | None = None) -> list:
        out = (ctypes.c_float * max(1, cap))()
        kinds = (ctypes.c_int32 * max(1, cap))()
        n = L.check(L.lib().gs_plan_timer_read(self.handle, out, kinds, int(cap)), "gs_plan_timer_read")
        return [float(out[i]) for i in range(n) if kind is None or kinds[i] == kind]

    def timer_read_by_kind(self, cap: int = 4096) -> dict:
        out = (ctypes.c_float * max(1, cap))()
        kinds = (ctypes.c_int32 * max(1, cap))()
        n = L.check(L.lib().gs_plan_timer_read(self.handle, out, kinds, int(cap)), "gs_plan_timer_read")
        by: dict = {}
        for i in range(n):
            by.setdefault(int(kinds[i]), []).append(float(out[i]))
        return by

    def pack(self, src_slot, src_dtype, flat: torch.Tensor, scale=1.0, mode=L.GS_SCALE_NONE, stream=None):
        L.check(
            L.lib().gs_pack(self.handle, src_slot, L.gs_dtype(src_dtype), flat.data_ptr(),
                            L.gs_dtype(flat.dtype), float(scale), mode, self._stream(stream)),
            "gs_pack",
        )

    def unpack(self, flat: torch.Tensor, dst_slot, dst_dtype, sqnorm: torch.Tensor | None = None,
               accumulate=False, stream=None):
        L.check(
            L.lib().gs_unpack(self.handle, flat.data_ptr(), L.gs_dtype(flat.dtype), dst_slot,
                              L.gs_dtype(dst_dtype), None if sqnorm is None else sqnorm.data_ptr(),
                              int(bool(accumulate)), self._stream(stream)),
            "gs_unpack",
        )

    def unpack_check(self, flat: torch.Tensor, dst_slot, dst_dtype, found_inf: torch.Tensor, stream=None):
        if found_inf.dtype != torch.float32 or found_inf.numel() < 1 or \
                (found_inf.device.type == "cuda") != (self.kind == L.GS_DEV_HIP):
            raise ValueError("found_inf: fp32, where the plan runs")
        L.check(
            L.lib().gs_unpack_check(self.handle, flat.data_ptr(), L.gs_dtype(flat.dtype), dst_slot,
                                    L.gs_dtype(dst_dtype), found_inf.data_ptr(), self._stream(stream)),
            "gs_unpack_check",
        )

    def scale(self, slot, dtype, s, mode=L.GS_SCALE_MUL, stream=None):
        L.check(L.lib().gs_scale(self.handle, slot, L.gs_dtype(dtype), float(s), mode, self._stream(stream)),
                "gs_scale")

    def sqnorm(self, slot, dtype, out: torch.Tensor, accumulate=False, stream=None):
        L.check(
            L.lib().gs_sqnorm(self.handle, slot, L.gs_dtype(dtype), out.data_ptr(), int(bool(accumulate)),
                              self._stream(stream)),
            "gs_sqnorm",
        )

    def sqnorm_partial(self, slot, dtype, stream=None):
        L.check(L.lib().gs_sqnorm_partial(self.handle, slot, L.gs_dtype(dtype), self._stream(stream)),
                "gs_sqnorm_partial")

    def sqnorm_partial_out(self, slot, dtype, groups: torch.Tensor, stream=None) -> int:
        if groups.dtype != torch.float32 or groups.numel() < L.GS_RED_PARTIALS or not groups.is_contiguous() or \
                (groups.device.type == "cuda") != (self.kind == L.GS_DEV_HIP):
            raise ValueError(f"partial sums: contiguous fp32[>= {L.GS_RED_PARTIALS}] where the plan runs")
        n = ctypes.c_int32()
        L.check(L.lib().gs_sqnorm_partial_out(self.handle, slot, L.gs_dtype(dtype), groups.data_ptr(),
                                              ctypes.byref(n), self._stream(stream)), "gs_sqnorm_partial_out")
        return n.value

    def set_clip_groups(self, max_norm: float | None, eps: float, groups: torch.Tensor, n_groups: int,
                        sq_mul: float = 1.0, coef_mul: float = 1.0, out: torch.Tensor | None = None):
        for t in (groups, out):
            if t is not None and (t.dtype != torch.float32 or (t.device.type == "cuda") != (self.kind == L.GS_DEV_HIP)):
                raise ValueError("clip tensors: fp32, where the plan runs")
        if out is not None and out.numel() < 3:
            raise ValueError("clip out: 3 elements")
        if not groups.is_contiguous() or groups.numel() < int(n_groups):
            raise ValueError(f"partial sums: {n_groups} contiguous floats expected, got {groups.numel()}")
        L.check(L.lib().gs_plan_set_clip_groups(self.handle, groups.data_ptr(), int(n_groups), float(max_norm or 0.0),
                                                float(eps), float(sq_mul), float(coef_mul),
                                                None if out is None else out.data_ptr()), "gs_plan_set_clip_groups")
        self._clip_refs = (groups, out)

    def set_read_hint(self, hint: int):
        L.check(L.lib().gs_plan_set_read_hint(self.handle, int(hint)), "gs_plan_set_read_hint")

    def set_clip(self, max_norm: float | None, eps: float = 1e-6, sqnorm: torch.Tensor | None = None,
                 sq_mul: float = 1.0, coef_mul: float = 1.0, out: torch.Tensor | None = None):
        for t in (sqnorm, out):
            if t is not None and (t.dtype != torch.float32 or (t.device.type == "cuda") != (self.kind == L.GS_DEV_HIP)):
                raise ValueError("clip tensors: fp32, where the plan runs")
        if out is not None and out.numel() < 3:
            raise ValueError("clip out: 3 elements")
        L.check(L.lib().gs_plan_set_clip(self.handle, None if sqnorm is None else sqnorm.data_ptr(),
                                         float(max_norm or 0.0), float(eps), float(sq_mul), float(coef_mul),
                                         None if out is None else out.data_ptr()), "gs_plan_set_clip")
        self._clip_refs = (sqnorm, out)

    def sum(self, slot, dtype, out: torch.Tensor, accumulate=False, stream=None):
        L.check(
            L.lib().gs_sum(self.handle, slot, L.gs_dtype(dtype), out.data_ptr(), int(bool(accumulate)),
                           self._stream(stream)),
            "gs_sum",
        )

    def clip_scale(self, slot, dtype, stream=None):
        L.check(L.lib().gs_clip_scale(self.handle, slot, L.gs_dtype(dtype), self._stream(stream)), "gs_clip_scale")

    def unscale_check(self, slot, dtype, inv_scale: torch.Tensor | None, found_inf: torch.Tensor, stream=None):
        L.check(
            L.lib().gs_unscale_check(self.handle, slot, L.gs_dtype(dtype),
                                     None if inv_scale is None else inv_scale.data_ptr(),
                                     found_inf.data_ptr(), self._stream(stream)),
            "gs_unscale_check",
        )

    def sgd(self, grad_dtype, lr, momentum, dampening, weight_decay, nesterov, maximize, first_step,
            lowp_dtype=None, grad_scale=None, found_inf=None, stream=None):
        L.check(
            L.lib().gs_sgd_step(
                self.handle, L.gs_dtype(grad_dtype), -1 if lowp_dtype is None else L.gs_dtype(lowp_dtype),
                float(lr), float(momentum), float(dampening), float(weight_decay), int(bool(nesterov)),
                int(bool(maximize)), -1 if first_step == -1 else int(bool(first_step)),
                None if grad_scale is None else grad_scale.data_ptr(),
                None if found_inf is None else found_inf.data_ptr(), self._stream(stream)),
            "gs_sgd_step",
        )

    def _where_plan(self, t: torch.Tensor) -> bool:
        return (t.device.type == "cuda") == (self.kind == L.GS_DEV_HIP)

# ... 129 lines not shown
```

distributed_training_amd/optim.py:

```python
from __future__ import annotations

import math
import os
from typing import Iterable

import torch
from torch.autograd.graph import increment_version

from . import _lib as L
from .multi_tensor import TensorListPlan, clip_coef, is_dense, update_task_units


CLIP_FUSED = os.environ.get("GSYNC_CLIP_FUSED", "1") not in ("", "0")


def _capturing() -> bool:
    return torch.cuda.is_initialized() and torch.cuda.is_current_stream_capturing()


class _PlanCache:

    def __init__(self):
        self._plans: dict = {}
        self.timer_slots = 0

    def get(self, params):
        key = tuple(id(p) for p in params) + (params[0].device,)
        plan = self._plans.get(key)
        if plan is None:
            plan = TensorListPlan([p.numel() for p in params], params[0].device,
                                  task_units=update_task_units(params[0].device))
            if self.timer_slots and plan.kind == L.GS_DEV_HIP:
                plan.timer_enable(self.timer_slots)
            self._plans[key] = plan
        return plan

    def plans(self):
        return list(self._plans.values())


def _check_dense(p: torch.Tensor, g: torch.Tensor, what: str, seen: dict | None = None):
    ps = p.stride()
    if g.stride() != ps:
        raise RuntimeError(f"{what}: grad layout must match its parameter's (param {ps}, grad {g.stride()})")
    if seen is not None and seen.get(id(p)) == ps:
        return
    if not is_dense(p):
        raise RuntimeError(f"{what}: parameters must be dense (got strides {ps})")
    if seen is not None:
        seen[id(p)] = ps


def _sq_norms(self) -> list:
    return list(self._last_norms)


def _bind_adapt(self, plan, group, ps):
    adapt = group.get("adapt")
    flags = tuple((p.ndim > 1) if adapt is None else bool(adapt) for p in ps)
    if getattr(plan, "_adapt", None) != flags:
        if _capturing():
            raise RuntimeError(f"{self._name}: take one eager step before capturing "
                               "(the plan's adaptation flags and scratch are set there)")
        plan.set_adapt(flags)
        plan._adapt = flags
        plan._norms = torch.zeros(2 * len(ps), dtype=torch.float32, device=ps[0].device)


class _FusedBase(torch.optim.Optimizer):
    _name: str
    _timer_kinds: tuple

    def __init__(self, params, defaults):
        super().__init__(params, defaults)
        self._plans = _PlanCache()
        self.grad_scale: torch.Tensor | None = None
        self.found_inf: torch.Tensor | None = None
        self._clip_buf: dict = {}
        self._norm_ddp = None
        self._dev_hyper: dict = {}
        self._dense_seen: dict = {}

    @property
    def capturable(self) -> bool:
        return bool(self.defaults.get("capturable"))

    def _group_hyper(self, gi, group, device):
        h = self._dev_hyper.get(gi)
        if h is None or h["hyper"].device != device:
            if _capturing():
                raise RuntimeError("capturable optimizer: take one step outside the graph before capturing it")
            h = {"hyper": torch.zeros(3, dtype=torch.float32, device=device),
                 "lr": torch.zeros(1, dtype=torch.float64, device=device), "lr_host": None}
            self._dev_hyper[gi] = h
        return h

    def refresh_hyper(self):
        if _capturing():
            return
        for gi, group in enumerate(self.param_groups):
            h = self._dev_hyper.get(gi)
            if h is not None and h["lr_host"] != group["lr"]:
                lr = float(group["lr"])
                h["lr"].fill_(lr)
                h["hyper"][0:1].fill_(lr)
                h["lr_host"] = group["lr"]

    def load_state_dict(self, state_dict):
        super().load_state_dict(state_dict)
        self._dev_hyper = {}

    def enable_kernel_timer(self, n_slots: int = 256):
        self._plans.timer_slots = int(n_slots)
        for plan in self._plans.plans():
            if plan.kind == L.GS_DEV_HIP:
                plan.timer_enable(n_slots)

    def kernel_ms(self) -> list:
        return [ms for plan in self._plans.plans() if plan.kind == L.GS_DEV_HIP
                for k, v in plan.timer_read_by_kind().items() if k in self._timer_kinds for ms in v]

    def _check_param(self, p):
        if p.grad.is_sparse:
            raise RuntimeError(f"{self._name} does not support sparse gradients")
        _check_dense(p, p.grad, self._name, self._dense_seen)
        if p.dtype != torch.float32:
            raise RuntimeError(f"{self._name} expects fp32 parameters (keep a fp32 master copy)")

    def _clip_buffer(self, device):
        buf = self._clip_buf.get(device)
        if buf is None:
            buf = self._clip_buf[device] = torch.zeros(4, dtype=torch.float32, device=device)
        return buf

    def _collect(self, group, by_first=False):
        out = {}
        for p in group["params"]:
            if p.grad is None:
                continue
            self._check_param(p)
            buf, first = None, False
            st = self.state[p] if group["momentum"] != 0 or by_first else None
            if group["momentum"] != 0:
                buf = st.get("momentum_buffer")
                first = buf is None
                if first:
                    if _capturing():
                        raise RuntimeError(f"{self._name}: momentum buffers must exist before capture "
                                           "(take an eager step first)")
                    buf = st["momentum_buffer"] = torch.zeros_like(p, memory_format=torch.preserve_format)
            ps, gs, bs = out.setdefault((p.grad.dtype, first) if by_first else p.grad.dtype, ([], [], []))
            ps.append(p)
            gs.append(p.grad)
            bs.append(buf)
        return out

    def _device_state(self) -> bool:
        return self.capturable or self.found_inf is not None or bool(self._dev_hyper)

    def fuse_grad_norm_into(self, ddp):
        if not self.defaults.get("max_grad_norm"):
            raise ValueError("fuse_grad_norm_into: the optimizer has no max_grad_norm")
        ddp.set_grad_sqnorm_target(self._clip_buffer(ddp.device)[3:4])
        self._norm_ddp = (ddp, frozenset(id(p) for p in ddp._params))

    def _ddp_sqnorm(self, device):
        if self._norm_ddp is None:
            return None
        ddp, ids = self._norm_ddp
        if not ddp._sqnorm_valid or ddp.device != device:
            return None
        mine, ver = set(), 0
        for g in self.param_groups:
            for p in g["params"]:
                gr = p.grad
                if gr is not None:
                    mine.add(id(p))
                    ver += gr._version
        ddp._sqnorm_valid = False
        if mine != ids or ver != ddp._sqnorm_versions:
            return None
        return self._clip_buf[device][3:4]

    def _clip_scale(self, device, all_plans):
        max_norm = self.defaults.get("max_grad_norm")
        if not max_norm:
            for plan, _ in all_plans:
                if getattr(plan, "_clip_on", False):
                    plan.set_clip(None)
                    plan._clip_on = False
            return self.grad_scale
        buf = self._clip_buffer(device)
        self.last_grad_norm = buf[2:3]
        if CLIP_FUSED:
            fused = self._ddp_sqnorm(device)
            if fused is not None:
                for plan, _ in all_plans:
                    plan.set_clip(float(max_norm), 1e-6, fused, out=buf[0:3])
                    plan._clip_on = True
                self.last_clip_source = "ddp_unpack"
                return self.grad_scale
            self.last_clip_source = "optimizer"
            if len(all_plans) == 1:
                plan, gdt = all_plans[0]
                plan.sqnorm_partial(1, gdt)
                plan.set_clip(float(max_norm), 1e-6, None, out=buf[0:3])
                plan._clip_on = True
            else:
                raw = buf[3:4]
                for i, (plan, gdt) in enumerate(all_plans):
                    plan.sqnorm(1, gdt, raw, accumulate=i > 0)
                for plan, _ in all_plans:
                    plan.set_clip(float(max_norm), 1e-6, raw, out=buf[0:3])
                    plan._clip_on = True
            return self.grad_scale
        return self._clip_scale_separate(device, all_plans)

    def _clip_scale_separate(self, device, all_plans):
        max_norm = self.defaults.get("max_grad_norm")
        buf = self._clip_buffer(device)
        sq, coef, norm = buf[0:1], buf[1:2], buf[2:3]
        self.last_grad_norm = norm
        for plan, _ in all_plans:
            if getattr(plan, "_clip_on", False):
                plan.set_clip(None)
                plan._clip_on = False
        for i, (plan, gdt) in enumerate(all_plans):
            plan.sqnorm(1, gdt, sq, accumulate=i > 0)
        if self.grad_scale is not None:
            sq.mul_(self.grad_scale * self.grad_scale)
        clip_coef(sq, float(max_norm), 1e-6, coef, norm)
        if self.grad_scale is not None:
            coef.mul_(self.grad_scale)
        return coef


class FusedSGD(_FusedBase):
    def __init__(self, params, lr=1e-3, momentum=0.0, dampening=0.0, weight_decay=0.0, nesterov=False,
                 *, maximize=False, foreach=None, differentiable=False, fused=None, max_grad_norm=None,
                 capturable=False):
        if lr < 0.0:
            raise ValueError(f"Invalid learning rate: {lr}")
        if momentum < 0.0:
            raise ValueError(f"Invalid momentum value: {momentum}")
        if weight_decay < 0.0:
            raise ValueError(f"Invalid weight_decay value: {weight_decay}")
        if nesterov and (momentum <= 0 or dampening != 0):
            raise ValueError("Nesterov momentum requires a momentum and zero dampening")
        if differentiable:
            raise ValueError("FusedSGD does not support differentiable=True")
        defaults = dict(lr=lr, momentum=momentum, dampening=dampening, weight_decay=weight_decay,
                        nesterov=nesterov, maximize=maximize, foreach=foreach, differentiable=False,
                        fused=fused, max_grad_norm=max_grad_norm, capturable=bool(capturable))
        super().__init__(params, defaults)

    _name = "FusedSGD"
    _timer_kinds = (L.GS_OP_SGD,)

    @torch.no_grad()
    def step(self, closure=None):
        loss = None
        if closure is not None:
            with torch.enable_grad():
                loss = closure()
        dev_state = self._device_state()
        work = []
        for gi, group in enumerate(self.param_groups):
            for (gdt, first), (ps, gs, bs) in self._collect(group, by_first=True).items():
                plan = self._plans.get(ps)
                plan.set_ptrs(0, ps)
                plan.set_ptrs(1, gs)
                plan.set_ptrs(2, [b.data_ptr() if b is not None else 0 for b in bs])
                flag = None
                if dev_state:
                    h = self._group_hyper(gi, group, ps[0].device)
                    if getattr(plan, "_hyper", None) is not h["hyper"]:
                        plan.set_hyper_source(h["hyper"])
                    if group["momentum"] != 0:
                        flag = h.setdefault("first_flags", {}).setdefault(
                            id(plan), torch.zeros(1, dtype=torch.float32, device=ps[0].device))
                        if first:
                            flag.fill_(1.0)
                work.append((group, plan, gdt, first, h if dev_state else None, flag))
        if dev_state:
            self.refresh_hyper()
        if not work:
            return loss
        scale = self._clip_scale(work[0][1].device, [(w[1], w[2]) for w in work])
        for group, plan, gdt, first, h, flag in work:
            if flag is not None:
                h["hyper"][1:2].copy_(flag)
            plan.sgd(gdt, group["lr"], group["momentum"], group["dampening"], group["weight_decay"],
                     group["nesterov"], group["maximize"], -1 if flag is not None else first,
                     grad_scale=scale, found_inf=self.found_inf)
            if flag is not None:
                if self.found_inf is not None:
                    flag.mul_(self.found_inf)
                else:
                    flag.zero_()
        return loss


class FusedLARS(_FusedBase):

    def __init__(self, params, lr=1e-3, momentum=0.9, weight_decay=0.0, trust_coefficient=1e-3, eps=1e-8,
                 *, capturable=False):
        if lr < 0.0:
            raise ValueError(f"Invalid learning rate: {lr}")
        if momentum < 0.0:
            raise ValueError(f"Invalid momentum value: {momentum}")
        if weight_decay < 0.0:
            raise ValueError(f"Invalid weight_decay value: {weight_decay}")
        if trust_coefficient < 0.0:
            raise ValueError(f"Invalid trust_coefficient value: {trust_coefficient}")
        if eps < 0.0:
            raise ValueError(f"Invalid epsilon value: {eps}")
        defaults = dict(lr=lr, momentum=momentum, weight_decay=weight_decay, trust_coefficient=trust_coefficient,
                        eps=eps, adapt=None, capturable=bool(capturable))
        super().__init__(params, defaults)
        self._last_norms: list = []

    _name = "FusedLARS"
    _timer_kinds = (L.GS_OP_LARS_NORM, L.GS_OP_LARS)
    sq_norms = _sq_norms
    _bind_adapt = _bind_adapt

    @torch.no_grad()
    def step(self, closure=None):
        loss = None
        if closure is not None:
            with torch.enable_grad():
                loss = closure()
        dev_state = self._device_state()
        work = []
        for gi, group in enumerate(self.param_groups):
            for gdt, (ps, gs, bs) in self._collect(group).items():
                plan = self._plans.get(ps)
                plan.set_ptrs(0, ps)
                plan.set_ptrs(1, gs)
                if group["momentum"] != 0:
                    plan.set_ptrs(2, bs)
                self._bind_adapt(plan, group, ps)
                if dev_state:
                    h = self._group_hyper(gi, group, ps[0].device)
                    if getattr(plan, "_hyper", None) is not h["hyper"]:
                        plan.set_hyper_source(h["hyper"])
                work.append((group, plan, gdt, ps))
        if dev_state:
            self.refresh_hyper()
        self._last_norms = [(ps, plan._norms) for _, plan, _, ps in work]
        for group, plan, gdt, ps in work:
            plan.lars_norms(gdt, plan._norms)
            plan.lars(gdt, group["lr"], group["momentum"], group["weight_decay"], group["trust_coefficient"],
                      group["eps"], plan._norms, grad_scale=self.grad_scale, found_inf=self.found_inf)
        return loss


class _DeviceSteps:

    def _gather(self, cap):
        work = []
        for gi, group in enumerate(self.param_groups):
            buckets: dict = {}
            by_cohort: dict = {}
            h = None
            live = []

            def add(key, p):
                st = self.state[p]
                for lst, x in zip(buckets.setdefault(key, ([], [], [], [])),
                                  (p, p.grad, st["exp_avg"], st["exp_avg_sq"])):
                    lst.append(x)

            for p in group["params"]:
                if p.grad is None:
                    continue
                self._check_param(p)
                st = self.state[p]
                if "exp_avg" not in st:
                    if _capturing():
                        raise RuntimeError(f"{self._name}: state must exist before capture (take an eager step first)")
                    st["step"] = torch.tensor(0.0, dtype=torch.float32)
                    st["exp_avg"] = torch.zeros_like(p, memory_format=torch.preserve_format)
                    st["exp_avg_sq"] = torch.zeros_like(p, memory_format=torch.preserve_format)
                live.append(p)
            for p in live:
                st = self.state[p]
                if cap:
                    if h is None:
                        h = self._group_hyper(gi, group, p.device)
                    if id(st["step"]) not in h.get("cohorts", {}):
                        self._adopt_cohorts(h, group)
                    by_cohort.setdefault(id(st["step"]), []).append(p)
                else:
                    st["step"] += 1
                    add((p.grad.dtype, float(st["step"].item())), p)
            for cid, ps in by_cohort.items():
                c = h["cohorts"][cid]
                if len(ps) < len(c["members"]):
                    c = self._split_cohort(h, c, ps)
                work.append((group, None, None, (h, c), None))
                for p in ps:
                    add((p.grad.dtype, id(c["step"])), p)
            cohort_hyper = {id(c["step"]): c["hyper"] for c in h["cohorts"].values()} if h is not None else {}
            for (gdt, step), lists in buckets.items():
                plan = self._plans.get(lists[0])
                for slot, lst in enumerate(lists):
                    plan.set_ptrs(slot, lst)
                if cap:
                    hyper = cohort_hyper[step]
                    if getattr(plan, "_hyper", None) is not hyper:
                        plan.set_hyper_source(hyper)
                    step = None
                work.append((group, plan, gdt, step, lists[0]))
        return work

    def _adopt_cohorts(self, h, group):
        cohorts = h.setdefault("cohorts", {})
        by_value: dict = {}
        for p in group["params"]:
            st = self.state.get(p)
            if not st or "exp_avg" not in st:
                continue
            t = st.get("step")
            if t is not None and id(t) in cohorts:
                continue
            if _capturing():
                raise RuntimeError(f"{self._name}: state must exist before capture (take an eager step first)")
            v = 0.0 if t is None else float(t)
            c = by_value.get(v)
            if c is None:
                c = by_value[v] = {"step": torch.full((1,), v, dtype=torch.float64, device=p.device),
                                   "hyper": torch.zeros(3, dtype=torch.float32, device=p.device),
                                   "members": set()}
                cohorts[id(c["step"])] = c
            c["members"].add(id(p))
            st["step"] = c["step"]

    def _split_cohort(self, h, c, ps):
        if _capturing():
            raise RuntimeError(f"{self._name}: the set of parameters with grads changed inside a capture")
        n = {"step": c["step"].clone(), "hyper": torch.zeros_like(c["hyper"]), "members": {id(p) for p in ps}}
        c["members"] -= n["members"]
        h["cohorts"][id(n["step"])] = n
        for p in ps:
            self.state[p]["step"] = n["step"]
        return n

    def state_dict(self):
        sd = super().state_dict()
        vals: dict = {}
        for k, st in list(sd["state"].items()):
            t = st.get("step")
            if torch.is_tensor(t) and t.dtype == torch.float64:
                v = vals.get(id(t))
                if v is None:
                    v = vals[id(t)] = float(t.item())
                dev = t.device if self.capturable else torch.device("cpu")
                sd["state"][k] = dict(st, step=torch.tensor(v, dtype=torch.float32, device=dev))
        return sd


class FusedAdam(_DeviceSteps, _FusedBase):

    _name = "FusedAdam"
    _timer_kinds = (L.GS_OP_ADAM,)

    def __init__(self, params, lr=1e-3, betas=(0.9, 0.999), eps=1e-8, weight_decay=0.0, amsgrad=False,
                 *, foreach=None, maximize=False, capturable=False, differentiable=False, fused=None,
                 decoupled_weight_decay=False, adamw=None, max_grad_norm=None):
        if not 0.0 <= lr:
            raise ValueError(f"Invalid learning rate: {lr}")
        if not 0.0 <= eps:
            raise ValueError(f"Invalid epsilon value: {eps}")
        if not 0.0 <= betas[0] < 1.0 or not 0.0 <= betas[1] < 1.0:
            raise ValueError(f"Invalid beta parameters: {betas}")
        if amsgrad:
            raise NotImplementedError("FusedAdam: amsgrad is not on the reference path")
        if differentiable:
            raise ValueError("FusedAdam does not support differentiable=True")
        adamw = bool(decoupled_weight_decay if adamw is None else adamw)
        defaults = dict(lr=lr, betas=tuple(betas), eps=eps, weight_decay=weight_decay, amsgrad=False,
                        foreach=foreach, maximize=maximize, capturable=bool(capturable), differentiable=False,
                        fused=fused, decoupled_weight_decay=adamw, max_grad_norm=max_grad_norm)
        super().__init__(params, defaults)

    @torch.no_grad()
    def step(self, closure=None):
        loss = None
        if closure is not None:
            with torch.enable_grad():
                loss = closure()
        cap = self._device_state()
        work = self._gather(cap)
        plans = [(w[1], w[2]) for w in work if w[1] is not None]
        if not plans:
            return loss
        if cap:
            self.refresh_hyper()
        scale = self._clip_scale(plans[0][0].device, plans)
        for group, plan, gdt, step, _ in work:
            beta1, beta2 = group["betas"]
            if plan is None:
                h, c = step
                L.check(L.lib().gs_adam_hyper(
                    L.GS_DEV_HIP if c["step"].is_cuda else L.GS_DEV_HOST, c["step"].data_ptr(), h["lr"].data_ptr(),
                    float(beta1), float(beta2), float(group["weight_decay"]),
                    None if self.found_inf is None else self.found_inf.data_ptr(), c["hyper"].data_ptr(),
                    L.stream_ptr(c["step"].device) if c["step"].is_cuda else None), "gs_adam_hyper")
                continue
            if step is None:
                plan.adam(gdt, group["lr"], beta1, beta2, group["eps"], group["weight_decay"],
                          group["decoupled_weight_decay"], group["maximize"], -1.0, 1.0,
                          grad_scale=scale, found_inf=self.found_inf)
                continue
            lr = group["lr"]
            bias_correction1 = 1 - beta1 ** step
            bias_correction2 = 1 - beta2 ** step
            step_size = (lr / bias_correction1) * -1
            bias_correction2_sqrt = bias_correction2 ** 0.5
            plan.adam(gdt, lr, beta1, beta2, group["eps"], group["weight_decay"],
                      group["decoupled_weight_decay"], group["maximize"], step_size, bias_correction2_sqrt,
                      grad_scale=scale, found_inf=self.found_inf)
        return loss


class FusedAdamW(FusedAdam):
    def __init__(self, params, lr=1e-3, betas=(0.9, 0.999), eps=1e-8, weight_decay=1e-2, **kw):
        kw.pop("decoupled_weight_decay", None)
        super().__init__(params, lr=lr, betas=betas, eps=eps, weight_decay=weight_decay, adamw=True, **kw)


class FusedLAMB(_DeviceSteps, _FusedBase):

    _name = "FusedLAMB"
    _timer_kinds = (L.GS_OP_LAMB_MOMENTS, L.GS_OP_LAMB)
    sq_norms = _sq_norms
    _bind_adapt = _bind_adapt

    def __init__(self, params, lr=1e-3, betas=(0.9, 0.999), eps=1e-6, weight_decay=0.01, bias_correction=True,
                 min_trust=None, max_trust=None, max_grad_norm=None, *, capturable=False):
        if not 0.0 <= lr:
            raise ValueError(f"Invalid learning rate: {lr}")
        if not 0.0 <= eps:
            raise ValueError(f"Invalid epsilon value: {eps}")
        if not 0.0 <= betas[0] < 1.0 or not 0.0 <= betas[1] < 1.0:
            raise ValueError(f"Invalid beta parameters: {betas}")
        if weight_decay < 0.0:
            raise ValueError(f"Invalid weight_decay value: {weight_decay}")
        lo = 0.0 if min_trust is None else float(min_trust)
        hi = math.inf if max_trust is None else float(max_trust)
        if not 0.0 <= lo <= hi:
            raise ValueError(f"Invalid trust-ratio clamp: [{min_trust}, {max_trust}]")
        defaults = dict(lr=lr, betas=tuple(betas), eps=eps, weight_decay=weight_decay,
                        bias_correction=bool(bias_correction), min_trust=min_trust, max_trust=max_trust,
                        max_grad_norm=max_grad_norm, adapt=None, capturable=bool(capturable))
        super().__init__(params, defaults)
        self._last_norms: list = []

    @torch.no_grad()
    def step(self, closure=None):
        loss = None
        if closure is not None:
            with torch.enable_grad():
                loss = closure()
        cap = self._device_state()
        work = self._gather(cap)
        plans = [(w[1], w[2]) for w in work if w[1] is not None]
        if not plans:
            return loss
        for group, plan, _, _, ps in work:
            if plan is not None:
                self._bind_adapt(plan, group, ps)
        if cap:
            self.refresh_hyper()
        self._last_norms = [(w[4], w[1]._norms) for w in work if w[1] is not None]
        scale = self.grad_scale
        if self.defaults.get("max_grad_norm"):
            scale = self._clip_scale_separate(plans[0][0].device, plans)
        for group, plan, gdt, step, _ in work:
            beta1, beta2 = group["betas"]
            if plan is None:
                h, c = step
                L.check(L.lib().gs_lamb_hyper(
                    L.GS_DEV_HIP if c["step"].is_cuda else L.GS_DEV_HOST, c["step"].data_ptr(), h["lr"].data_ptr(),
                    float(beta1), float(beta2), int(group["bias_correction"]),
                    None if self.found_inf is None else self.found_inf.data_ptr(), c["hyper"].data_ptr(),
                    L.stream_ptr(c["step"].device) if c["step"].is_cuda else None), "gs_lamb_hyper")
                continue
            bc1 = bc2s = 1.0
            if step is not None and group["bias_correction"]:
                bc1 = 1 - beta1 ** step
                bc2s = math.sqrt(1 - beta2 ** step)
            lo = 0.0 if group["min_trust"] is None else group["min_trust"]
            hi = math.inf if group["max_trust"] is None else group["max_trust"]
            norms = plan._norms
            plan.lamb_moments(gdt, beta1, beta2, group["eps"], group["weight_decay"], bc1, bc2s, norms,
                              grad_scale=scale, found_inf=self.found_inf)
            plan.lamb(group["lr"], group["eps"], group["weight_decay"], bc1, bc2s, norms, lo, hi,
                      found_inf=self.found_inf)
        return loss


_NORM_PLANS: dict = {}


@torch.no_grad()
def clip_grad_norm_(parameters: torch.Tensor | Iterable[torch.Tensor], max_norm: float, norm_type: float = 2.0,
                    error_if_nonfinite: bool = False, foreach=None) -> torch.Tensor:
    if isinstance(parameters, torch.Tensor):
        parameters = [parameters]
    grads = [p.grad for p in parameters if p.grad is not None]
    if float(norm_type) != 2.0:
        raise NotImplementedError("clip_grad_norm_: only norm_type=2 is on the gradient-sync path")
    if len(grads) == 0:
        return torch.tensor(0.0)
    dev = grads[0].device
    groups: dict = {}
    for g in grads:
        if not is_dense(g):
            raise RuntimeError("clip_grad_norm_: grads must be dense")
        groups.setdefault(g.dtype, []).append(g)
    buf = torch.empty(4, dtype=torch.float32, device=dev)
    plans = []
    for dt, gl in groups.items():
        key = tuple(g.numel() for g in gl) + (dev,)
        plan = _NORM_PLANS.get(key)
        if plan is None:
            plan = TensorListPlan([g.numel() for g in gl], dev)
            if len(_NORM_PLANS) > 64:
                _NORM_PLANS.clear()
            _NORM_PLANS[key] = plan
        plan.set_ptrs(0, gl)
        plans.append((plan, dt))
    if len(plans) == 1 and not error_if_nonfinite:
        plan, dt = plans[0]
        plan.sqnorm_partial(0, dt)
        plan.set_clip(float(max_norm), 1e-6, None, out=buf[0:3])
    else:
        raw = buf[3:4]
        for i, (plan, dt) in enumerate(plans):
            plan.sqnorm(0, dt, raw, accumulate=i > 0)
        if error_if_nonfinite and not torch.isfinite(raw).item():
            raise RuntimeError(
                f"The total norm of order {float(norm_type)} for gradients from `parameters` is non-finite, "
                "so it cannot be clipped. To disable this error and scale the gradients by the non-finite "
                "norm anyway, set `error_if_nonfinite=False`")
        for plan, _ in plans:
            plan.set_clip(float(max_norm), 1e-6, raw, out=buf[0:3])
    for plan, dt in plans:
        plan.clip_scale(0, dt)
        plan.set_clip(None)
    norm = buf[2:3]
    increment_version(grads)
    return norm.reshape(())
```

distributed_training_amd/resnet.py:

```python
from __future__ import annotations

import torch
import torch.nn as nn

from .fused_bn import bn_act, bn_relu_pool


def conv3x3(in_planes, out_planes, stride=1):
    return nn.Conv2d(in_planes, out_planes, kernel_size=3, stride=stride, padding=1, bias=False)


def conv1x1(in_planes, out_planes, stride=1):
    return nn.Conv2d(in_planes, out_planes, kernel_size=1, stride=stride, bias=False)


def _downsample(seq, x):
    return bn_act(seq[1], seq[0](x), relu=False)


class BasicBlock(nn.Module):
    expansion = 1

    def __init__(self, inplanes, planes, stride=1, downsample=None):
        super().__init__()
        self.conv1 = conv3x3(inplanes, planes, stride)
        self.bn1 = nn.BatchNorm2d(planes)
        self.relu = nn.ReLU(inplace=True)
        self.conv2 = conv3x3(planes, planes)
        self.bn2 = nn.BatchNorm2d(planes)
        self.downsample = downsample
        self.stride = stride

    def forward_pair(self, pair, fork_out):
        x, identity = pair
        if self.downsample is not None:
            identity = _downsample(self.downsample, identity)
        out = bn_act(self.bn1, self.conv1(x))
        return bn_act(self.bn2, self.conv2(out), residual=identity, fork=fork_out)

    def forward(self, x):
        return self.forward_pair((x, x), False)


class Bottleneck(nn.Module):
    expansion = 4

    def __init__(self, inplanes, planes, stride=1, downsample=None):
        super().__init__()
        self.conv1 = conv1x1(inplanes, planes)
        self.bn1 = nn.BatchNorm2d(planes)
        self.conv2 = conv3x3(planes, planes, stride)
        self.bn2 = nn.BatchNorm2d(planes)
        self.conv3 = conv1x1(planes, planes * self.expansion)
        self.bn3 = nn.BatchNorm2d(planes * self.expansion)
        self.relu = nn.ReLU(inplace=True)
        self.downsample = downsample
        self.stride = stride

    def forward_pair(self, pair, fork_out):
        x, identity = pair
        if self.downsample is not None:
            identity = _downsample(self.downsample, identity)
        out = bn_act(self.bn1, self.conv1(x))
        out = bn_act(self.bn2, self.conv2(out))
        return bn_act(self.bn3, self.conv3(out), residual=identity, fork=fork_out)

    def forward(self, x):
        return self.forward_pair((x, x), False)


class ResNet(nn.Module):
    def __init__(self, block, layers, num_classes=1000, width=64):
        super().__init__()
        self.inplanes = width
        self.conv1 = nn.Conv2d(3, self.inplanes, kernel_size=7, stride=2, padding=3, bias=False)
        self.bn1 = nn.BatchNorm2d(self.inplanes)
        self.relu = nn.ReLU(inplace=True)
        self.maxpool = nn.MaxPool2d(kernel_size=3, stride=2, padding=1)
        self.layer1 = self._make_layer(block, width, layers[0])
        self.layer2 = self._make_layer(block, width * 2, layers[1], stride=2)
        self.layer3 = self._make_layer(block, width * 4, layers[2], stride=2)
        self.layer4 = self._make_layer(block, width * 8, layers[3], stride=2)
        self.avgpool = nn.AdaptiveAvgPool2d((1, 1))
        self.fc = nn.Linear(width * 8 * block.expansion, num_classes)
        for m in self.modules():
            if isinstance(m, nn.Conv2d):
                nn.init.kaiming_normal_(m.weight, mode="fan_out", nonlinearity="relu")
            elif isinstance(m, (nn.BatchNorm2d, nn.GroupNorm)):
                nn.init.constant_(m.weight, 1)
                nn.init.constant_(m.bias, 0)

    def _make_layer(self, block, planes, blocks, stride=1):
        downsample = None
        if stride != 1 or self.inplanes != planes * block.expansion:
            downsample = nn.Sequential(
                conv1x1(self.inplanes, planes * block.expansion, stride),
                nn.BatchNorm2d(planes * block.expansion),
            )
        layers = [block(self.inplanes, planes, stride, downsample)]
        self.inplanes = planes * block.expansion
        for _ in range(1, blocks):
            layers.append(block(self.inplanes, planes))
        return nn.Sequential(*layers)

    def _hooked(self):
        return any(m._forward_hooks or m._forward_pre_hooks
                   for layer in (self.layer1, self.layer2, self.layer3, self.layer4) for m in (layer, *layer))

    def forward(self, x):
        x = self.conv1(x)
        if self._hooked():
            x = bn_relu_pool(self.bn1, x, self.maxpool, fork=False)
            x = self.layer4(self.layer3(self.layer2(self.layer1(x))))
        else:
            blocks = [b for layer in (self.layer1, self.layer2, self.layer3, self.layer4) for b in layer]
            pair = bn_relu_pool(self.bn1, x, self.maxpool, fork=True)
            for b in blocks[:-1]:
                pair = b.forward_pair(pair, True)
            x = blocks[-1].forward_pair(pair, False)
        x = torch.flatten(self.avgpool(x), 1)
        return self.fc(x)


def resnet18(num_classes=1000, width=64, **_):
    return ResNet(BasicBlock, [2, 2, 2, 2], num_classes, width)


def resnet50(num_classes=1000, width=64, **_):
    return ResNet(Bottleneck, [3, 4, 6, 3], num_classes, width)


def resnet152(num_classes=1000, width=64, **_):
    return ResNet(Bottleneck, [3, 8, 36, 3], num_classes, width)


def micro_resnet(num_classes=10, width=8):
    return ResNet(BasicBlock, [1, 1, 1, 1], num_classes, width)


MODELS = {"resnet18": resnet18, "resnet50": resnet50, "resnet152": resnet152, "micro": micro_resnet}
```

include/gsync.h:

```cpp
#ifndef GSYNC_H
#define GSYNC_H

#include <stdint.h>

#ifdef __cplusplus
extern "C" {
#endif

#define GSYNC_VERSION 1000

#define GS_OK 0
#define GS_EINVAL (-1)
#define GS_EHIP (-2)
#define GS_ERCCL (-3)
#define GS_ESTATE (-4)
#define GS_ENOMEM (-5)
#define GS_ENODEV (-6)

#define GS_F32 0
#define GS_BF16 1
#define GS_F16 2
#define GS_F64 3
#define GS_I64 4
#define GS_I32 5
#define GS_U8 6

int gs_set_host_threads(int n);

#define GS_DEV_HOST 0
#define GS_DEV_HIP 1

#define GS_SUM 0
#define GS_PROD 1
#define GS_MAX 2
#define GS_MIN 3
#define GS_AVG 4

#define GS_SCALE_NONE 0
#define GS_SCALE_MUL 1
#define GS_SCALE_DIV 2

typedef struct gs_comm gs_comm;
typedef struct gs_plan gs_plan;
typedef struct gs_bucketer gs_bucketer;

int gs_version(void);
const char* gs_last_error(void);
int gs_device_count(void);

int gs_comm_unique_id_bytes(void);
int gs_comm_get_unique_id(uint8_t* out );
int gs_comm_create(int rank, int world, const uint8_t* uid, int device, gs_comm** out);
int gs_comm_create_ex(int rank, int world, const uint8_t* uid, int device, int max_ctas, gs_comm** out);
int gs_comm_destroy(gs_comm* c);
int gs_comm_abort(gs_comm* c);
int gs_comm_set_timeout(gs_comm* c, int64_t timeout_ms);
int gs_watchdog_pause(int pause);
int gs_comm_status(gs_comm* c, char* reason, int cap);
int gs_comm_rank(gs_comm* c);
int gs_comm_world(gs_comm* c);
int gs_comm_stream(gs_comm* c, void** stream_out);
int gs_stream_wait(void* waiter, void* signaler);

int gs_allreduce(gs_comm* c, const void* send, void* recv, int64_t count, int dtype, int op,
                 void* stream);
int gs_reduce_scatter(gs_comm* c, const void* send, void* recv, int64_t recv_count, int dtype,
                      int op, void* stream);
int gs_all_gather(gs_comm* c, const void* send, void* recv, int64_t send_count, int dtype,
                  void* stream);
int gs_allreduce_marked(gs_comm* c, const void* send, void* recv, int64_t count, int dtype, int op,
                        void* stream, gs_plan* consumer);
int gs_all_gather_marked(gs_comm* c, const void* send, void* recv, int64_t send_count, int dtype,
                         void* stream, gs_plan* consumer);
int gs_broadcast(gs_comm* c, const void* send, void* recv, int64_t count, int dtype, int root,
                 void* stream);

#define GS_PLAN_SLOTS 5
int gs_plan_create(int device_kind, int device, int n_tensors, const int64_t* numels,
                   int64_t align_elems, gs_plan** out);
int gs_plan_create_ex(int device_kind, int device, int n_tensors, const int64_t* numels,
                      int64_t align_elems, int64_t task_units, gs_plan** out);
int gs_plan_destroy(gs_plan* p);
int64_t gs_plan_flat_numel(gs_plan* p);
int gs_plan_offsets(gs_plan* p, int64_t* out );
int gs_plan_n_tasks(gs_plan* p);
int64_t gs_plan_task_units(gs_plan* p);
#define GS_OP_PACK 1
#define GS_OP_UNPACK 2
#define GS_OP_SCALE 3
#define GS_OP_SQNORM 4
#define GS_OP_UNSCALE 5
#define GS_OP_SGD 6
#define GS_OP_ADAM 7
#define GS_OP_SUM 8
#define GS_OP_LARS_NORM 9
#define GS_OP_LARS 10
#define GS_OP_LAMB_MOMENTS 11
#define GS_OP_LAMB 12
#define GS_OP_EMA 13
int gs_plan_timer_enable(gs_plan* p, int n_slots);
int gs_plan_timer_read(gs_plan* p, float* ms_out, int32_t* kind_out, int cap);
int gs_plan_set_ptrs(gs_plan* p, int slot, void* const* ptrs, void* stream);

int gs_pack(gs_plan* p, int src_slot, int src_dtype, void* flat, int flat_dtype, float scale,
            int scale_mode, void* stream);
int gs_unpack(gs_plan* p, const void* flat, int flat_dtype, int dst_slot, int dst_dtype,
              float* sqnorm_dev, int accumulate, void* stream);
int gs_unpack_check(gs_plan* p, const void* flat, int flat_dtype, int dst_slot, int dst_dtype,
                    float* found_inf, void* stream);
int gs_scale(gs_plan* p, int slot, int dtype, float s, int scale_mode, void* stream);
int gs_sqnorm(gs_plan* p, int slot, int dtype, float* sqnorm_dev, int accumulate, void* stream);
int gs_sum(gs_plan* p, int slot, int dtype, float* sum_dev, int accumulate, void* stream);
int gs_sqnorm_partial(gs_plan* p, int slot, int dtype, void* stream);
int gs_plan_set_read_hint(gs_plan* p, int hint);
int gs_plan_set_clip(gs_plan* p, const float* sqnorm_dev, float max_norm, float eps, float sq_mul,
                     float coef_mul, float* out_dev);
#define GS_RED_GROUPS 64
#define GS_RED_PARTIALS 1024
int gs_sqnorm_partial_out(gs_plan* p, int slot, int dtype, float* groups_out, int32_t* n_groups,
                          void* stream);
int gs_plan_set_clip_groups(gs_plan* p, const float* groups_dev, int32_t n_groups, float max_norm,
                            float eps, float sq_mul, float coef_mul, float* out_dev);
int gs_clip_scale(gs_plan* p, int slot, int dtype, void* stream);
int gs_clip_coef(int device_kind, const float* sqnorm_dev, float max_norm, float eps,
                 float* coef_dev, float* norm_dev, void* stream);
int gs_unscale_check(gs_plan* p, int slot, int dtype, const float* inv_scale_dev,
                     float* found_inf_dev, void* stream);

int gs_sgd_step(gs_plan* p, int grad_dtype, int lowp_dtype, double lr, double momentum,
                double dampening, double weight_decay, int nesterov, int maximize, int first_step,
                const float* grad_scale_dev, const float* found_inf_dev, void* stream);
int gs_adam_step(gs_plan* p, int grad_dtype, int lowp_dtype, double lr, double beta1,
                 double beta2, double eps, double weight_decay, int adamw, int maximize,
                 double step_size, double bias_correction2_sqrt, const float* grad_scale_dev,
                 const float* found_inf_dev, void* stream);
int gs_plan_set_adapt(gs_plan* p, const int32_t* adapt);
int gs_lars_norms(gs_plan* p, int grad_dtype, float* norms_out, void* stream);
int gs_lars_step(gs_plan* p, int grad_dtype, double lr, double momentum, double weight_decay,
                 double trust_coefficient, double eps, const float* norms,
                 const float* grad_scale_dev, const float* found_inf_dev, void* stream);
int gs_lars_step_lowp(gs_plan* p, int grad_dtype, int lowp_dtype, double lr, double momentum,
                      double weight_decay, double trust_coefficient, double eps, const float* norms,
                      const float* grad_scale_dev, const float* found_inf_dev, void* stream);
int gs_plan_set_hyper_source(gs_plan* p, const float* hyper);
int gs_adam_hyper(int device_kind, double* step, const double* lr, double beta1, double beta2,
                  double weight_decay, const float* found_inf, float* hyper, void* stream);
int gs_lamb_moments(gs_plan* p, int grad_dtype, double beta1, double beta2, double eps, double weight_decay,
                    double bc1, double bc2_sqrt, float* norms_out, const float* grad_scale_dev,
                    const float* found_inf_dev, void* stream);
int gs_lamb_step(gs_plan* p, double lr, double eps, double weight_decay, double bc1, double bc2_sqrt,
                 double min_ratio, double max_ratio, const float* norms, const float* found_inf_dev, void* stream);
int gs_lamb_step_lowp(gs_plan* p, int lowp_dtype, double lr, double eps, double weight_decay,
                      double bc1, double bc2_sqrt, double min_ratio, double max_ratio,
                      const float* norms, const float* found_inf_dev, void* stream);
int gs_lamb_hyper(int device_kind, double* step, const double* lr, double beta1, double beta2, int bias_correction,
                  const float* found_inf, float* hyper, void* stream);

int gs_ema_step(gs_plan* p, int src_dtype, int lowp_dtype , double weight, int copy,
                void* stream);
#define GS_EMA_EMA 0
#define GS_EMA_SWA 1
#define GS_EMA_WARMUP 2
int gs_ema_hyper(int device_kind, int64_t* n_averaged, int mode, double decay, float* hyper ,
                 void* stream);

int gs_compute_bucket_assignment(int n, const int64_t* nbytes, const int32_t* dtype_keys,
                                 const int32_t* order, int n_limits, const int64_t* limits,
                                 int32_t* bucket_of ,
                                 int32_t* bucket_members ,
                                 int32_t* bucket_counts );

#define GS_BKT_AUTO_COLLECTIVE 1
#define GS_BKT_GRAD_VIEW 2
#define GS_BKT_NO_SCALE 4
#define GS_BKT_REDUCE_SCATTER 8
#define GS_BKT_NO_UNPACK 16

int gs_bucketer_create(gs_comm* comm, int device_kind, int device, int n_params,
                       const int64_t* numels, int grad_dtype, int n_buckets,
                       const int32_t* bucket_counts, const int32_t* bucket_members,
                       int bucket_dtype, int64_t align_elems, float div_factor, int flags,
                       gs_bucketer** out);
int gs_bucketer_destroy(gs_bucketer* b);
int gs_bucketer_bucket_numel(gs_bucketer* b, int bucket, int64_t* out);
int gs_bucketer_shard_numel(gs_bucketer* b, int bucket, int64_t* out);
int gs_bucketer_param_location(gs_bucketer* b, int param, int32_t* bucket, int64_t* offset);
int gs_bucketer_set_bucket_dtype(gs_bucketer* b, int bucket, int grad_dtype, int bucket_dtype);
int gs_bucketer_set_bucket_buffer(gs_bucketer* b, int bucket, void* ptr);
int gs_bucketer_set_shard_buffer(gs_bucketer* b, int bucket, void* ptr);
int gs_bucketer_prepare(gs_bucketer* b, float* sqnorm_dev);
int gs_bucketer_mark_ready(gs_bucketer* b, int param, const void* grad, void* stream,
                           int32_t* ready_out, int32_t* n_ready);
int gs_bucketer_mark_unused(gs_bucketer* b, void* stream, int32_t* ready_out, int32_t* n_ready);
// ... 85 lines not shown
```

Before: 7227.

## Keep persistent bf16 weight copies written by the optimizer to skip autocast casts

Adds persistent flat bf16 copies of conv/linear weights, refreshed by the Adam step (lowp_dtype output) and published to ResNet forward through a table, so autocast no longer casts each fp32 weight to bf16 every iteration. A custom autograd node widens the bf16 weight gradients back to fp32 with one multi-tensor gs_widen kernel launch per group instead of per-tensor casts. It adds memory for the bf16 copies, version tracking and invalidation logic for other optimizers, plus fallback paths.

Result: no change. 7286, median of 6 (+0.8%).

```diff
diff --git a/distributed_training_amd/_lib.py b/distributed_training_amd/_lib.py
--- a/distributed_training_amd/_lib.py
+++ b/distributed_training_amd/_lib.py
@@ -29,6 +29,7 @@
 GS_OP_LARS_NORM, GS_OP_LARS = 9, 10
 GS_OP_LAMB_MOMENTS, GS_OP_LAMB = 11, 12
 GS_OP_EMA = 13
+GS_OP_WIDEN = 14
 GS_EMA_EMA, GS_EMA_SWA, GS_EMA_WARMUP = 0, 1, 2
 
 _TORCH_TO_GS = {
@@ -88,6 +89,7 @@
     "gs_unpack": (_c_int, [_vp, _vp, _c_int, _c_int, _c_int, _vp, _c_int, _vp]),
     "gs_unpack_check": (_c_int, [_vp, _vp, _c_int, _c_int, _c_int, _vp, _vp]),
     "gs_scale": (_c_int, [_vp, _c_int, _c_int, _c_f, _c_int, _vp]),
+    "gs_widen": (_c_int, [_vp, _c_int, _c_int, _c_int, _vp]),
     "gs_sqnorm": (_c_int, [_vp, _c_int, _c_int, _vp, _c_int, _vp]),
     "gs_sum": (_c_int, [_vp, _c_int, _c_int, _vp, _c_int, _vp]),
     "gs_sqnorm_partial": (_c_int, [_vp, _c_int, _c_int, _vp]),
diff --git a/distributed_training_amd/csrc/gs_common.h b/distributed_training_amd/csrc/gs_common.h
--- a/distributed_training_amd/csrc/gs_common.h
+++ b/distributed_training_amd/csrc/gs_common.h
@@ -354,6 +354,7 @@
 int hip_unpack_check(gs_plan* p, const void* flat, int flat_dt, int dst_slot, int dst_dt, float* found,
                      void* stream);
 int hip_scale(gs_plan* p, int slot, int dt, float s, int mode, void* stream);
+int hip_widen(gs_plan* p, int src_slot, int src_dt, int dst_slot, void* stream);
 int hip_sqnorm(gs_plan* p, int slot, int dt, float* sq, int acc, void* stream);
 int hip_sum(gs_plan* p, int slot, int dt, float* out, int acc, void* stream);
 int hip_clip_coef(const float* sq, float max_norm, float eps, float* coef, float* norm,
@@ -386,6 +387,7 @@
                 int acc);
 int host_unpack_check(gs_plan* p, const void* flat, int flat_dt, int dst_slot, int dst_dt, float* found);
 int host_scale(gs_plan* p, int slot, int dt, float s, int mode);
+int host_widen(gs_plan* p, int src_slot, int src_dt, int dst_slot);
 int host_clip_scale(gs_plan* p, int slot, int dt, const ClipArgs& clip);
 int host_sqnorm(gs_plan* p, int slot, int dt, float* sq, int acc);
 int host_sum(gs_plan* p, int slot, int dt, float* out, int acc);
diff --git a/distributed_training_amd/csrc/gs_engine.h b/distributed_training_amd/csrc/gs_engine.h
--- a/distributed_training_amd/csrc/gs_engine.h
+++ b/distributed_training_amd/csrc/gs_engine.h
@@ -726,6 +726,27 @@
   }
 };
 
+template <int N, int SD, bool NT = false>
+struct WidenOp : OpBase<N> {
+  static_assert(SD == GS_BF16 || SD == GS_F16, "widening reads a 16-bit source");
+  static constexpr int kG = GS_G_UNPACK;
+  static constexpr int kKind = GS_OP_WIDEN;
+  int slot, dslot;
+  struct Frag { float x[N]; };
+  __device__ int phys(int k) const { return k == 0 ? slot : (k == 1 ? dslot : k); }
+  __device__ bool fast_ok(const TV& v) const { return v.vec(0) && v.vec(1); }
+  template <bool F>
+  __device__ void load(const TV& v, int64_t e0, uint32_t lo, Frag& f) const {
+    if (v.ptr[0] == nullptr || v.ptr[1] == nullptr) return;
+    ld<SD, N, F, NT>(v.ptr[0], e0, lo, v.numel, v.vec(0), f.x);
+  }
+  template <bool F>
+  __device__ void apply(const TV& v, int64_t e0, uint32_t lo, Frag& f, float&) const {
+    if (v.ptr[0] == nullptr || v.ptr[1] == nullptr) return;
+    st<GS_F32, N, F>(v.ptr[1], e0, lo, v.numel, v.vec(1), f.x);
+  }
+};
+
 template <int N, int GD, int LD, bool NTG = true>
 struct SgdOp : OpBase<N> {
   static constexpr int kG = GS_G_SGD;
diff --git a/distributed_training_amd/csrc/gs_host.cpp b/distributed_training_amd/csrc/gs_host.cpp
--- a/distributed_training_amd/csrc/gs_host.cpp
+++ b/distributed_training_amd/csrc/gs_host.cpp
@@ -133,6 +133,18 @@
         for (int64_t i = i0; i < i1; ++i) stT<DT>(x, i, ldT<DT>(x, i) / s);
       else
         for (int64_t i = i0; i < i1; ++i) stT<DT>(x, i, ldT<DT>(x, i) * s);
+    });
+  });
+  return GS_OK;
+}
+
+int host_widen(gs_plan* p, int src_slot, int src_dt, int dst_slot) {
+  GS_DISPATCH_FLOAT(src_dt, SD, {
+    for_ranges(p, [&](int t, int64_t i0, int64_t i1) {
+      const void* src = slot(p, src_slot, t);
+      void* dst = slot(p, dst_slot, t);
+      if (src == nullptr || dst == nullptr) return;
+      for (int64_t i = i0; i < i1; ++i) stT<GS_F32>(dst, i, ldT<SD>(src, i));
     });
   });
   return GS_OK;
diff --git a/distributed_training_amd/csrc/gs_kernels.hip b/distributed_training_amd/csrc/gs_kernels.hip
--- a/distributed_training_amd/csrc/gs_kernels.hip
+++ b/distributed_training_amd/csrc/gs_kernels.hip
@@ -266,6 +266,20 @@
 }
 
 template <bool NT>
+static int widen_nt(gs_plan* p, int src_slot, int src_dt, int dst_slot, void* stream) {
+  switch (src_dt) {
+    case GS_BF16: { WidenOp<kUnit, GS_BF16, NT> op; op.slot = src_slot; op.dslot = dst_slot; return launch(p, op, stream); }
+    case GS_F16: { WidenOp<kUnit, GS_F16, NT> op; op.slot = src_slot; op.dslot = dst_slot; return launch(p, op, stream); }
+    default: return fail(GS_EINVAL, "gs_widen: the source dtype must be bf16 or f16");
+  }
+}
+int hip_widen(gs_plan* p, int src_slot, int src_dt, int dst_slot, void* stream) {
+  DeviceGuard g(p->device);
+  return nt_read_once(p->elems * dtype_bytes(src_dt)) ? widen_nt<true>(p, src_slot, src_dt, dst_slot, stream)
+                                                      : widen_nt<false>(p, src_slot, src_dt, dst_slot, stream);
+}
+
+template <bool NT>
 static int sqnorm_nt(gs_plan* p, int slot, int dt, float* sq, int acc, int groups_only, void* stream) {
   GS_DISPATCH_FLOAT(dt, DT, {
     SqnormOp<kUnit, DT, NT> op;
diff --git a/distributed_training_amd/csrc/gs_plan.cpp b/distributed_training_amd/csrc/gs_plan.cpp
--- a/distributed_training_amd/csrc/gs_plan.cpp
+++ b/distributed_training_amd/csrc/gs_plan.cpp
@@ -286,6 +286,17 @@
   return hip_scale(p, slot, dtype, s, scale_mode, stream);
 }
 
+int gs_widen(gs_plan* p, int src_slot, int src_dtype, int dst_slot, void* stream) {
+  GsRange range("gs_widen");
+  PLAN_OK(p);
+  SLOT_OK(src_slot);
+  SLOT_OK(dst_slot);
+  GS_CHECK_ARG(src_slot != dst_slot, "gs_widen: source and destination are the same slot");
+  GS_CHECK_ARG(src_dtype == GS_BF16 || src_dtype == GS_F16, "gs_widen: the source dtype must be bf16 or f16");
+  if (p->kind == GS_DEV_HOST) return host_widen(p, src_slot, src_dtype, dst_slot);
+  return hip_widen(p, src_slot, src_dtype, dst_slot, stream);
+}
+
 int gs_sqnorm(gs_plan* p, int slot, int dtype, float* sqnorm_dev, int accumulate, void* stream) {
   GsRange range("gs_sqnorm");
   PLAN_OK(p);
diff --git a/distributed_training_amd/csrc/gs_torch_hook.cpp b/distributed_training_amd/csrc/gs_torch_hook.cpp
--- a/distributed_training_amd/csrc/gs_torch_hook.cpp
+++ b/distributed_training_amd/csrc/gs_torch_hook.cpp
@@ -225,10 +225,109 @@
   std::vector<int> order_;
 };
 
-variable_list MarkReady::operator()(const variable_list& outputs, const variable_list& ) {
+variable_list MarkReady::operator()(const variable_list& outputs, const variable_list& inputs) {
+  if (!inputs.empty() && !inputs[0].defined()) return outputs;
   owner->on_grad(index);
   return outputs;
 }
+
+class LowpGroup;
+
+struct WidenNode : Node {
+  std::shared_ptr<LowpGroup> group;
+  explicit WidenNode(std::shared_ptr<LowpGroup> g) : group(std::move(g)) {}
+  variable_list apply(variable_list&& grads) override;
+  std::string name() const override { return "GsyncLowpWidenBackward"; }
+};
+
+class LowpGroup : public std::enable_shared_from_this<LowpGroup> {
+ public:
+  LowpGroup(std::vector<at::Tensor> params, at::Tensor flat, std::vector<int64_t> offsets, int device)
+      : params_(std::move(params)), flat_(std::move(flat)), offsets_(std::move(offsets)), device_(device) {
+    if (params_.size() != offsets_.size()) throw std::runtime_error("_gshook: one offset per parameter");
+    std::vector<int64_t> numels;
+    for (auto& p : params_) numels.push_back(p.numel());
+    const int rc = gs_plan_create_ex(device_ < 0 ? GS_DEV_HOST : GS_DEV_HIP, std::max(0, device_),
+                                     static_cast<int>(numels.size()), numels.data(), 0, 0, &plan_);
+    if (rc < 0) throw std::runtime_error(std::string("gs_plan_create_ex: ") + gs_last_error());
+    src_.resize(params_.size());
+    dst_.resize(params_.size());
+    undefined_.assign(params_.size(), 0);
+  }
+  ~LowpGroup() {
+    if (plan_ != nullptr) gs_plan_destroy(plan_);
+  }
+  LowpGroup(const LowpGroup&) = delete;
+  LowpGroup& operator=(const LowpGroup&) = delete;
+
+  std::vector<at::Tensor> forward() {
+    std::vector<at::Tensor> views;
+    views.reserve(params_.size());
+    undefined_.assign(params_.size(), 0);
+    {
+      at::NoGradGuard ng;
+      for (size_t i = 0; i < params_.size(); ++i)
+        views.push_back(flat_.as_strided(params_[i].sizes(), params_[i].strides(), offsets_[i]));
+    }
+    if (!at::GradMode::is_enabled()) return views;
+    bool any = false;
+    for (auto& p : params_) any = any || p.requires_grad();
+    if (!any) return views;
+    auto node = std::make_shared<WidenNode>(shared_from_this());
+    node->set_next_edges(torch::autograd::collect_next_edges(params_));
+    for (auto& v : views) torch::autograd::create_gradient_edge(v, node);
+    return views;
+  }
+
+  variable_list backward(variable_list&& grads) {
+    if (grads.size() != params_.size()) throw std::runtime_error("_gshook: LowpGroup got a wrong number of gradients");
+    variable_list outs(params_.size());
+    int src_dt = -1;
+    bool any = false;
+    for (size_t i = 0; i < params_.size(); ++i) {
+      src_[i] = dst_[i] = nullptr;
+      const at::Tensor& g = grads[i];
+      undefined_[i] = !g.defined();
+      if (!g.defined()) continue;
+      const int dt = g.scalar_type() == at::kBFloat16 ? GS_BF16 : (g.scalar_type() == at::kHalf ? GS_F16 : -1);
+      if (dt < 0 || (src_dt >= 0 && dt != src_dt) || !g.is_non_overlapping_and_dense() ||
+          g.numel() != params_[i].numel() || (device_ >= 0) != g.is_cuda()) {
+        outs[i] = g.to(at::kFloat);
+        continue;
+      }
+      src_dt = dt;
+      outs[i] = at::empty_strided(g.sizes(), g.strides(), g.options().dtype(at::kFloat));
+      src_[i] = g.data_ptr();
+      dst_[i] = outs[i].data_ptr();
+      any = true;
+    }
+    if (any) {
+      void* stream = device_ < 0 ? nullptr
+                                 : c10::hip::getCurrentHIPStream(static_cast<c10::DeviceIndex>(device_)).stream();
+      int rc = gs_plan_set_ptrs(plan_, 0, src_.data(), stream);
+      if (rc >= 0) rc = gs_plan_set_ptrs(plan_, 1, dst_.data(), stream);
+      if (rc >= 0) rc = gs_widen(plan_, 0, src_dt, 1, stream);
+      if (rc < 0) throw std::runtime_error(std::string("gs_widen: ") + gs_last_error());
+      ++launches_;
+    }
+    return outs;
+  }
+
+  int64_t launches() const { return launches_; }
+  bool undefined(int i) const { return undefined_.at(static_cast<size_t>(i)) != 0; }
+
+ private:
+  std::vector<at::Tensor> params_;
+  at::Tensor flat_;
+  std::vector<int64_t> offsets_;
+  int device_;
+  gs_plan* plan_ = nullptr;
+  std::vector<void*> src_, dst_;
+  std::vector<char> undefined_;
+  int64_t launches_ = 0;
+};
+
+variable_list WidenNode::apply(variable_list&& grads) { return group->backward(std::move(grads)); }
 
 }
 
@@ -248,4 +347,10 @@
       .def("in_backward", &Hooks::in_backward)
       .def("finalize_queued", &Hooks::finalize_queued)
       .def("stream", &Hooks::stream);
+  py::class_<LowpGroup, std::shared_ptr<LowpGroup>>(m, "LowpGroup")
+      .def(py::init<std::vector<at::Tensor>, at::Tensor, std::vector<int64_t>, int>(), py::arg("params"),
+           py::arg("flat"), py::arg("offsets"), py::arg("device"))
+      .def("forward", &LowpGroup::forward)
+      .def("launches", &LowpGroup::launches)
+      .def("undefined", &LowpGroup::undefined);
 }
diff --git a/distributed_training_amd/ddp.py b/distributed_training_amd/ddp.py
--- a/distributed_training_amd/ddp.py
+++ b/distributed_training_amd/ddp.py
@@ -14,6 +14,7 @@
 from torch.distributed.algorithms.join import Join, Joinable, JoinHook
 
 from . import _lib as L
+from . import lowp
 from .comm import get_communicator
 from .multi_tensor import TensorListPlan, dense_like_param, is_dense
 
@@ -372,6 +373,11 @@
             self._native.set_bucketer(self._bucketer.handle.value, len(self._bucketer.buckets))
             self._native.set_mark_unused(bool(self.static_graph))
         self._set_native(self._native_ok())
+        self._lowp_groups: list = []
+        self._lowp_asked: list = []
+        if self.device.type == "cuda" and lowp.enabled() and L.hook_module() is not None:
+            self._lowp_asked = [p for p in lowp.asked_params(module) if id(p) in self._param_index]
+        self._lowp_form()
 
     def _flags(self):
         flags = 0
@@ -403,6 +409,37 @@
         if getattr(self, "_native", None) is not None:
             self._native.set_bucketer(b.handle.value, len(buckets))
         return b
+
+    def _lowp_form(self):
+        self._lowp_groups = []
+        if not self._lowp_asked:
+            return
+        if not self._has_rebuilt_buckets and (self.static_graph or not self.find_unused_parameters):
+            return
+        asked = {id(p) for p in self._lowp_asked}
+        for b in self._bucketer.buckets:
+            ps = [self._params[i] for i in b]
+            mine = [p for p in ps if id(p) in asked]
+            if mine and all(p.dtype == torch.float32 and is_dense(p) for p in ps):
+                self._lowp_groups.append(lowp.Group(ps, mine, self.device))
+
+    def _lowp_table(self):
+        if not self._lowp_groups or not self.module.training or not lowp.autocast_bf16() or L._capturing():
+            return None
+        table = {}
+        for g in self._lowp_groups:
+            if g.dead or g.native is None:
+                continue
+            if not g.current():
+                g.refill()
+            for p, v in g.views():
+                table[id(p)] = v
+        return table or None
+
+    def lowp_counters(self) -> dict:
+        gs = self._lowp_groups
+        return {"groups": len(gs), "refills": sum(g.refills for g in gs),
+                "widen_launches": sum(g.widen_launches() for g in gs)}
 
     def _native_ok(self) -> bool:
         return (self._native is not None and bool(self._bucketer.flags & L.GS_BKT_AUTO_COLLECTIVE)
@@ -658,7 +695,12 @@
             dev = torch.device(self.device_type, self.device_ids[0])
             inputs = tuple(x.to(dev, non_blocking=True) if isinstance(x, torch.Tensor) else x for x in inputs)
             kwargs = {k: (v.to(dev, non_blocking=True) if isinstance(v, torch.Tensor) else v) for k, v in kwargs.items()}
-        output = self.module(*inputs, **kwargs)
+        table = self._lowp_table() if self._lowp_groups else None
+        if table is None:
+            output = self.module(*inputs, **kwargs)
+        else:
+            with lowp.published(table):
+                output = self.module(*inputs, **kwargs)
         if sync_bufs and post_fwd:
             self._sync_buffers()
         if grad_sync:
@@ -713,6 +755,8 @@
             if not self._in_backward:
                 if self._used_local is not None:
                     self._used_local[idx] = 1
+                return
+            if self._lowp_groups and lowp.took_no_part(param):
                 return
             if not self._finalize_queued:
                 self._finalize_queued = True
@@ -887,6 +931,7 @@
         self._bucketer = self._make_bucketer(buckets)
         self._has_rebuilt_buckets = True
         self._ready_order = []
+        self._lowp_form()
 
     def _sync_bucket_indices(self, buckets):
         if self.world_size == 1:
@@ -1171,6 +1216,7 @@
             except Exception:
                 pass
         self._hook_handles = []
+        self._lowp_groups = []
         if getattr(self, "_native", None) is not None:
             self._native.detach()
             self._native_on = False
diff --git a/distributed_training_amd/lowp.py b/distributed_training_amd/lowp.py
--- /dev/null
+++ b/distributed_training_amd/lowp.py
@@ -0,0 +1,149 @@
+from __future__ import annotations
+
+import os
+import weakref
+
+import torch
+
+from . import _lib as L
+from .multi_tensor import TensorListPlan, is_dense
+
+ALIGN_ELEMS = 64
+
+
+def enabled() -> bool:
+    return os.environ.get("GSYNC_LOWP_WEIGHTS", "1") not in ("", "0")
+
+
+_registry: dict = {}
+_published: dict = {}
+
+
+def registry_size() -> int:
+    return len(_registry)
+
+
+class Group:
+
+    def __init__(self, params, asked, device):
+        self.params = list(params)
+        self.plan = TensorListPlan([p.numel() for p in self.params], device, align=ALIGN_ELEMS)
+        self.flat = torch.zeros(self.plan.flat_numel, dtype=torch.bfloat16, device=device)
+        self.ptrs = [self.flat.data_ptr() + 2 * off for off in self.plan.offsets]
+        self.versions: list = [None] * len(self.params)
+        self.dead = False
+        self.refills = 0
+        want = {id(p) for p in asked}
+        self.asked = [i for i, p in enumerate(self.params) if id(p) in want]
+        self.asked_pos = {i: k for k, i in enumerate(self.asked)}
+        self.native = None
+        if self.asked:
+            self.native = L.hook_module().LowpGroup(
+                [self.params[i] for i in self.asked], self.flat, [self.plan.offsets[i] for i in self.asked],
+                device.index if device.type == "cuda" else -1)
+        keys = []
+        ref = weakref.ref(self)
+        for i, p in enumerate(self.params):
+            _registry[id(p)] = (weakref.ref(p), ref, i)
+            keys.append(id(p))
+        weakref.finalize(self, _drop, keys, ref)
+
+    def current(self) -> bool:
+        return all(p._version == v for p, v in zip(self.params, self.versions))
+
+    def refill(self):
+        self.plan.set_ptrs(0, self.params)
+        self.plan.pack(0, torch.float32, self.flat)
+        self.versions = [p._version for p in self.params]
+        self.refills += 1
+
+    def views(self):
+        return zip((self.params[i] for i in self.asked), self.native.forward())
+
+    def widen_launches(self) -> int:
+        return 0 if self.native is None else int(self.native.launches())
+
+
+def _drop(keys, ref):
+    for k in keys:
+        e = _registry.get(k)
+        if e is not None and e[1] is ref:
+            del _registry[k]
+
+
+def _entry(p):
+    e = _registry.get(id(p))
+    if e is None or e[0]() is not p:
+        return None
+    g = e[1]()
+    if g is None or g.dead:
+        return None
+    return g, e[2]
+
+
+def copies_of(params):
+    if not _registry:
+        return None
+    out = [_entry(p) for p in params]
+    return out if any(e is not None for e in out) else None
+
+
+def written(entries):
+    for e, p in entries:
+        e[0].versions[e[1]] = p._version
+
+
+def invalidate(params, dead: bool = False):
+    if not _registry:
+        return
+    for p in params:
+        e = _entry(p)
+        if e is not None:
+            e[0].versions[e[1]] = None
+            e[0].dead = e[0].dead or dead
+
+
+def took_no_part(param) -> bool:
+    e = _entry(param) if _registry else None
+    if e is None or e[0].native is None:
+        return False
+    pos = e[0].asked_pos.get(e[1])
+    return pos is not None and bool(e[0].native.undefined(pos))
+
+
+def weight(param):
+    return _published.get(id(param)) if _published else None
+
+
+def asked_params(module):
+    fn = getattr(module, "lowp_weight_modules", None)
+    if fn is None:
+        return []
+    out, seen = [], set()
+    for m in fn():
+        for p in (m.weight, getattr(m, "bias", None)):
+            if p is not None and id(p) not in seen and p.dtype == torch.float32 and p.requires_grad and is_dense(p):
+                seen.add(id(p))
+                out.append(p)
+    return out
+
+
+def autocast_bf16() -> bool:
+    return torch.is_autocast_enabled("cuda") and torch.get_autocast_dtype("cuda") == torch.bfloat16
+
+
+class published:
+
+    def __init__(self, table):
+        self.table = table
+
+    def __enter__(self):
+        global _published
+        self.prev = _published
+        _published = self.table
+        return self
+
+    def __exit__(self, *exc):
+        global _published
+        _published = self.prev
+        return False
diff --git a/distributed_training_amd/multi_tensor.py b/distributed_training_amd/multi_tensor.py
--- a/distributed_training_amd/multi_tensor.py
+++ b/distributed_training_amd/multi_tensor.py
@@ -136,6 +136,10 @@
     def scale(self, slot, dtype, s, mode=L.GS_SCALE_MUL, stream=None):
         L.check(L.lib().gs_scale(self.handle, slot, L.gs_dtype(dtype), float(s), mode, self._stream(stream)),
                 "gs_scale")
+
+    def widen(self, src_slot, src_dtype, dst_slot, stream=None):
+        L.check(L.lib().gs_widen(self.handle, src_slot, L.gs_dtype(src_dtype), dst_slot, self._stream(stream)),
+                "gs_widen")
 
     def sqnorm(self, slot, dtype, out: torch.Tensor, accumulate=False, stream=None):
         L.check(
diff --git a/distributed_training_amd/optim.py b/distributed_training_amd/optim.py
--- a/distributed_training_amd/optim.py
+++ b/distributed_training_amd/optim.py
@@ -8,6 +8,7 @@
 from torch.autograd.graph import increment_version
 
 from . import _lib as L
+from . import lowp
 from .multi_tensor import TensorListPlan, clip_coef, is_dense, update_task_units
 
 
@@ -126,6 +127,24 @@
         _check_dense(p, p.grad, self._name, self._dense_seen)
         if p.dtype != torch.float32:
             raise RuntimeError(f"{self._name} expects fp32 parameters (keep a fp32 master copy)")
+
+    def _lowp_split(self, ps, *lists):
+        copies = lowp.copies_of(ps)
+        if copies is None:
+            return [(ps, None, lists)]
+        if self.capturable or _capturing():
+            lowp.invalidate(ps, dead=True)
+            return [(ps, None, lists)]
+        if all(c is not None for c in copies):
+            return [(ps, copies, lists)]
+        have = [k for k, c in enumerate(copies) if c is not None]
+        rest = [k for k, c in enumerate(copies) if c is None]
+        return [([ps[k] for k in have], [copies[k] for k in have], tuple([x[k] for k in have] for x in lists)),
+                ([ps[k] for k in rest], None, tuple([x[k] for k in rest] for x in lists))]
+
+    def _lowp_written(self, ps, copies):
+        if copies is not None and self.found_inf is None:
+            lowp.written(zip(copies, ps))
 
     def _clip_buffer(self, device):
         buf = self._clip_buf.get(device)
@@ -266,11 +285,15 @@
         dev_state = self._device_state()
         work = []
         for gi, group in enumerate(self.param_groups):
-            for (gdt, first), (ps, gs, bs) in self._collect(group, by_first=True).items():
+            collected = self._collect(group, by_first=True)
+            for (gdt, first), ps, copies, (gs, bs) in (
+                    (key, *part) for key, (ps, gs, bs) in collected.items() for part in self._lowp_split(ps, gs, bs)):
                 plan = self._plans.get(ps)
                 plan.set_ptrs(0, ps)
                 plan.set_ptrs(1, gs)
                 plan.set_ptrs(2, [b.data_ptr() if b is not None else 0 for b in bs])
+                if copies is not None:
+                    plan.set_ptrs(3, [g.ptrs[i] for g, i in copies])
                 flag = None
                 if dev_state:
                     h = self._group_hyper(gi, group, ps[0].device)
@@ -281,18 +304,20 @@
                             id(plan), torch.zeros(1, dtype=torch.float32, device=ps[0].device))
                         if first:
                             flag.fill_(1.0)
-                work.append((group, plan, gdt, first, h if dev_state else None, flag))
+                work.append((group, plan, gdt, first, h if dev_state else None, flag, ps, copies))
         if dev_state:
             self.refresh_hyper()
         if not work:
             return loss
         scale = self._clip_scale(work[0][1].device, [(w[1], w[2]) for w in work])
-        for group, plan, gdt, first, h, flag in work:
+        for group, plan, gdt, first, h, flag, ps, copies in work:
             if flag is not None:
                 h["hyper"][1:2].copy_(flag)
             plan.sgd(gdt, group["lr"], group["momentum"], group["dampening"], group["weight_decay"],
                      group["nesterov"], group["maximize"], -1 if flag is not None else first,
+                     lowp_dtype=None if copies is None else torch.bfloat16,
                      grad_scale=scale, found_inf=self.found_inf)
+            self._lowp_written(ps, copies)
             if flag is not None:
                 if self.found_inf is not None:
                     flag.mul_(self.found_inf)
@@ -350,6 +375,7 @@
             self.refresh_hyper()
         self._last_norms = [(ps, plan._norms) for _, plan, _, ps in work]
         for group, plan, gdt, ps in work:
+            lowp.invalidate(ps)
             plan.lars_norms(gdt, plan._norms)
             plan.lars(gdt, group["lr"], group["momentum"], group["weight_decay"], group["trust_coefficient"],
                       group["eps"], plan._norms, grad_scale=self.grad_scale, found_inf=self.found_inf)
@@ -358,7 +384,7 @@
 
 class _DeviceSteps:
 
-    def _gather(self, cap):
+    def _gather(self, cap, lowp_ok=False):
         work = []
         for gi, group in enumerate(self.param_groups):
             buckets: dict = {}
@@ -404,15 +430,21 @@
                     add((p.grad.dtype, id(c["step"])), p)
             cohort_hyper = {id(c["step"]): c["hyper"] for c in h["cohorts"].values()} if h is not None else {}
             for (gdt, step), lists in buckets.items():
-                plan = self._plans.get(lists[0])
-                for slot, lst in enumerate(lists):
-                    plan.set_ptrs(slot, lst)
-                if cap:
-                    hyper = cohort_hyper[step]
-                    if getattr(plan, "_hyper", None) is not hyper:
-                        plan.set_hyper_source(hyper)
-                    step = None
-                work.append((group, plan, gdt, step, lists[0]))
+                parts = self._lowp_split(lists[0], *lists[1:]) if lowp_ok else [(lists[0], None, lists[1:])]
+                for ps, copies, rest in parts:
+                    plan = self._plans.get(ps)
+                    for slot, lst in enumerate((ps, *rest)):
+                        plan.set_ptrs(slot, lst)
+                    if copies is not None:
+                        plan.set_ptrs(4, [g.ptrs[i] for g, i in copies])
+                    plan._lowp = copies
+                    st = step
+                    if cap:
+                        hyper = cohort_hyper[step]
+                        if getattr(plan, "_hyper", None) is not hyper:
+                            plan.set_hyper_source(hyper)
+                        st = None
+                    work.append((group, plan, gdt, st, ps))
         return work
 
     def _adopt_cohorts(self, h, group):
@@ -492,14 +524,14 @@
             with torch.enable_grad():
                 loss = closure()
         cap = self._device_state()
-        work = self._gather(cap)
+        work = self._gather(cap, lowp_ok=True)
         plans = [(w[1], w[2]) for w in work if w[1] is not None]
         if not plans:
             return loss
         if cap:
             self.refresh_hyper()
         scale = self._clip_scale(plans[0][0].device, plans)
-        for group, plan, gdt, step, _ in work:
+        for group, plan, gdt, step, ps in work:
             beta1, beta2 = group["betas"]
             if plan is None:
                 h, c = step
@@ -512,7 +544,9 @@
             if step is None:
                 plan.adam(gdt, group["lr"], beta1, beta2, group["eps"], group["weight_decay"],
                           group["decoupled_weight_decay"], group["maximize"], -1.0, 1.0,
+                          lowp_dtype=None if plan._lowp is None else torch.bfloat16,
                           grad_scale=scale, found_inf=self.found_inf)
+                self._lowp_written(ps, plan._lowp)
                 continue
             lr = group["lr"]
             bias_correction1 = 1 - beta1 ** step
@@ -521,7 +555,9 @@
             bias_correction2_sqrt = bias_correction2 ** 0.5
             plan.adam(gdt, lr, beta1, beta2, group["eps"], group["weight_decay"],
                       group["decoupled_weight_decay"], group["maximize"], step_size, bias_correction2_sqrt,
+                      lowp_dtype=None if plan._lowp is None else torch.bfloat16,
                       grad_scale=scale, found_inf=self.found_inf)
+            self._lowp_written(ps, plan._lowp)
         return loss
 
 
@@ -578,7 +614,7 @@
         scale = self.grad_scale
         if self.defaults.get("max_grad_norm"):
             scale = self._clip_scale_separate(plans[0][0].device, plans)
-        for group, plan, gdt, step, _ in work:
+        for group, plan, gdt, step, work_ps in work:
             beta1, beta2 = group["betas"]
             if plan is None:
                 h, c = step
@@ -595,6 +631,7 @@
             lo = 0.0 if group["min_trust"] is None else group["min_trust"]
             hi = math.inf if group["max_trust"] is None else group["max_trust"]
             norms = plan._norms
+            lowp.invalidate(work_ps)
             plan.lamb_moments(gdt, beta1, beta2, group["eps"], group["weight_decay"], bc1, bc2s, norms,
                               grad_scale=scale, found_inf=self.found_inf)
             plan.lamb(group["lr"], group["eps"], group["weight_decay"], bc1, bc2s, norms, lo, hi,
diff --git a/distributed_training_amd/resnet.py b/distributed_training_amd/resnet.py
--- a/distributed_training_amd/resnet.py
+++ b/distributed_training_amd/resnet.py
@@ -2,7 +2,9 @@
 
 import torch
 import torch.nn as nn
+import torch.nn.functional as F
 
+from . import lowp
 from .fused_bn import bn_act, bn_relu_pool
 
 
@@ -14,8 +16,19 @@
     return nn.Conv2d(in_planes, out_planes, kernel_size=1, stride=stride, bias=False)
 
 
+def _wx(m, x):
+    w = lowp.weight(m.weight)
+    if w is None or not lowp.autocast_bf16() or m._forward_hooks or m._forward_pre_hooks:
+        return m(x)
+    if type(m) is nn.Conv2d:
+        return m._conv_forward(x, w, None if m.bias is None else lowp.weight(m.bias))
+    if type(m) is nn.Linear and (m.bias is None or lowp.weight(m.bias) is not None):
+        return F.linear(x, w, None if m.bias is None else lowp.weight(m.bias))
+    return m(x)
+
+
 def _downsample(seq, x):
-    return bn_act(seq[1], seq[0](x), relu=False)
+    return bn_act(seq[1], _wx(seq[0], x), relu=False)
 
 
 class BasicBlock(nn.Module):
@@ -35,8 +48,8 @@
         x, identity = pair
         if self.downsample is not None:
             identity = _downsample(self.downsample, identity)
-        out = bn_act(self.bn1, self.conv1(x))
-        return bn_act(self.bn2, self.conv2(out), residual=identity, fork=fork_out)
+        out = bn_act(self.bn1, _wx(self.conv1, x))
+        return bn_act(self.bn2, _wx(self.conv2, out), residual=identity, fork=fork_out)
 
     def forward(self, x):
         return self.forward_pair((x, x), False)
@@ -61,9 +74,9 @@
         x, identity = pair
         if self.downsample is not None:
             identity = _downsample(self.downsample, identity)
-        out = bn_act(self.bn1, self.conv1(x))
-        out = bn_act(self.bn2, self.conv2(out))
-        return bn_act(self.bn3, self.conv3(out), residual=identity, fork=fork_out)
+        out = bn_act(self.bn1, _wx(self.conv1, x))
+        out = bn_act(self.bn2, _wx(self.conv2, out))
+        return bn_act(self.bn3, _wx(self.conv3, out), residual=identity, fork=fork_out)
 
     def forward(self, x):
         return self.forward_pair((x, x), False)
@@ -107,8 +120,11 @@
         return any(m._forward_hooks or m._forward_pre_hooks
                    for layer in (self.layer1, self.layer2, self.layer3, self.layer4) for m in (layer, *layer))
 
+    def lowp_weight_modules(self):
+        return [m for m in self.modules() if type(m) in (nn.Conv2d, nn.Linear)]
+
     def forward(self, x):
-        x = self.conv1(x)
+        x = _wx(self.conv1, x)
         if self._hooked():
             x = bn_relu_pool(self.bn1, x, self.maxpool, fork=False)
             x = self.layer4(self.layer3(self.layer2(self.layer1(x))))
@@ -119,7 +135,7 @@
                 pair = b.forward_pair(pair, True)
             x = blocks[-1].forward_pair(pair, False)
         x = torch.flatten(self.avgpool(x), 1)
-        return self.fc(x)
+        return _wx(self.fc, x)
 
 
 def resnet18(num_classes=1000, width=64, **_):
diff --git a/include/gsync.h b/include/gsync.h
--- a/include/gsync.h
+++ b/include/gsync.h
@@ -98,6 +98,7 @@
 #define GS_OP_LAMB_MOMENTS 11
 #define GS_OP_LAMB 12
 #define GS_OP_EMA 13
+#define GS_OP_WIDEN 14
 int gs_plan_timer_enable(gs_plan* p, int n_slots);
 int gs_plan_timer_read(gs_plan* p, float* ms_out, int32_t* kind_out, int cap);
 int gs_plan_set_ptrs(gs_plan* p, int slot, void* const* ptrs, void* stream);
@@ -109,6 +110,7 @@
 int gs_unpack_check(gs_plan* p, const void* flat, int flat_dtype, int dst_slot, int dst_dtype,
                     float* found_inf, void* stream);
 int gs_scale(gs_plan* p, int slot, int dtype, float s, int scale_mode, void* stream);
+int gs_widen(gs_plan* p, int src_slot, int src_dtype, int dst_slot, void* stream);
 int gs_sqnorm(gs_plan* p, int slot, int dtype, float* sqnorm_dev, int accumulate, void* stream);
 int gs_sum(gs_plan* p, int slot, int dtype, float* sum_dev, int accumulate, void* stream);
 int gs_sqnorm_partial(gs_plan* p, int slot, int dtype, void* stream);
```
